# robertknight/ocrs

Measured on AMD Instinct MI355X. Metric: pages/sec end-to-end (1024x1024), higher is better.
Workload: dtype f32

## Files before the change

### include/ocrs_amd.h

```cpp
#ifndef OCRS_AMD_H
#define OCRS_AMD_H

#include <stddef.h>
#include <stdint.h>

#if defined(__GNUC__)
#define OCRS_API __attribute__((visibility("default")))
#else
#define OCRS_API
#endif

#ifdef __cplusplus
extern "C" {
#endif

typedef enum ocrs_status {
    OCRS_OK = 0,
    OCRS_ERR_INVALID_ARGUMENT = 1,
    OCRS_ERR_MODEL_NOT_LOADED = 2,
    OCRS_ERR_MODEL_DIMS = 3,
    OCRS_ERR_RUN_FAILED = 4,
    OCRS_ERR_WRONG_OUTPUT = 5,
    OCRS_ERR_IMAGE_SOURCE = 6,
    OCRS_ERR_DEVICE = 7,
// ... 258 lines not shown

typedef struct ocrs_speckle_params {
    float threshold;
    int32_t max_area;
    int32_t max_hole;
    int32_t keep_near;
    float paper;
    float ink_level;
} ocrs_speckle_params;
typedef struct ocrs_speckle_info {
    int32_t paper_bin;
    int32_t ink_bin;
    float paper_fill;
    float ink_fill;
    uint64_t ink;
    uint64_t counted;
    uint64_t specks;
    uint64_t kept;
    uint64_t speck_pixels;
    uint64_t kept_pixels;
    uint64_t holes;
    uint64_t hole_pixels;
} ocrs_speckle_info;
OCRS_API ocrs_status ocrs_speckle_params_default(ocrs_speckle_params* out);
OCRS_API ocrs_status ocrs_speckle_params_check(const ocrs_speckle_params* params);
OCRS_API ocrs_status ocrs_engine_despeckle_page(const ocrs_engine* e, const ocrs_page* page, const ocrs_speckle_params* params,
                                                ocrs_page** out_page, uint8_t** out_mask, ocrs_speckle_info* out_info);
OCRS_API ocrs_status ocrs_engine_despeckle_pages(const ocrs_engine* e, const ocrs_page* const* pages, size_t n,
                                                 const ocrs_speckle_params* params, ocrs_page** out_pages, uint8_t** out_masks,
                                                 ocrs_speckle_info* out_infos);

OCRS_API float ocrs_engine_detection_threshold(const ocrs_engine* e);

OCRS_API ocrs_status ocrs_engine_find_text_lines(const ocrs_engine* e, const ocrs_page* page, const float* word_rects,
                                        size_t n_words, float** line_rects, size_t** line_offsets,
                                        size_t* n_lines);

OCRS_API ocrs_status ocrs_engine_find_text_lines_batch(const ocrs_engine* e, size_t n_pages, const float* word_rects,
                                                       const size_t* word_offsets, float** line_rects,
                                                       size_t** line_offsets, size_t** page_line_offsets);

OCRS_API ocrs_status ocrs_engine_find_text_lines_indexed(const ocrs_engine* e, const ocrs_page* page, const float* word_rects,
                                                         size_t n_words, float** line_rects, size_t** line_offsets,
                                                         size_t* n_lines, size_t** word_index);
OCRS_API ocrs_status ocrs_engine_find_text_lines_batch_indexed(const ocrs_engine* e, size_t n_pages, const float* word_rects,
                                                               const size_t* word_offsets, float** line_rects,
                                                               size_t** line_offsets, size_t** page_line_offsets,
                                                               size_t** word_index);

typedef struct ocrs_text_char {
    uint32_t ch;
    int32_t top, left, bottom, right;
} ocrs_text_char;

OCRS_API ocrs_status ocrs_engine_recognize_text(const ocrs_engine* e, const ocrs_page* page, const float* line_rects,
                                       const size_t* line_offsets, size_t n_lines, ocrs_text_char** chars,
                                       size_t** char_offsets);
OCRS_API ocrs_status ocrs_engine_recognize_text_batch(const ocrs_engine* e, const ocrs_page* const* pages, size_t n_pages,
                                             const size_t* page_line_offsets, const float* line_rects,
                                             const size_t* line_offsets, size_t n_lines,
                                             ocrs_text_char** chars, size_t** char_offsets);

OCRS_API ocrs_status ocrs_engine_recognize_text_scored(const ocrs_engine* e, const ocrs_page* page, const float* line_rects,
                                                       const size_t* line_offsets, size_t n_lines, ocrs_text_char** chars,
                                                       size_t** char_offsets, float** char_logp, double** line_score);
OCRS_API ocrs_status ocrs_engine_recognize_text_batch_scored(const ocrs_engine* e, const ocrs_page* const* pages,
                                                             size_t n_pages, const size_t* page_line_offsets,
                                                             const float* line_rects, const size_t* line_offsets,
                                                             size_t n_lines, ocrs_text_char** chars, size_t** char_offsets,
                                                             float** char_logp, double** line_score);

OCRS_API ocrs_status ocrs_engine_recognize_tokens(const ocrs_engine* e, const ocrs_page* page, const float* line_rects,
                                         const size_t* line_offsets, size_t n_lines, uint32_t** labels,
                                         uint32_t** positions, size_t** token_offsets);

OCRS_API ocrs_status ocrs_engine_recognize_logits(const ocrs_engine* e, const ocrs_page* page, const float* line_rects,
                                         const size_t* line_offsets, size_t n_lines, float** logp, size_t** row_offsets,
                                         int* classes);

OCRS_API ocrs_status ocrs_engine_run_recognition_ops(const ocrs_engine* e, const int32_t* line_widths, size_t n_lines, int first_op,
                                                     int last_op, int gx_only, const float* input, size_t input_len, float** out,
                                                     size_t** out_offsets, int32_t** out_shapes);

OCRS_API ocrs_status ocrs_text_item_rotated_rect(const int32_t* rects_tlbr, size_t n_chars, float out6[6]);
OCRS_API ocrs_status ocrs_rotated_rect_corners(const float rect6[6], float out8[8]);

OCRS_API ocrs_status ocrs_engine_prepare_recognition_input(const ocrs_engine* e, const ocrs_page* page, const float* line,
                                                  size_t n_words, float** out, int* height, int* width);

OCRS_API ocrs_status ocrs_line_frame(const float* words, size_t n_words, int rec_height, double axis[2], double extents[4],
                                     uint32_t* resized_width, float coef[6], int32_t* ranges, int* empty);
OCRS_API ocrs_status ocrs_line_char_boxes(const float* words, size_t n_words, int rec_height, uint32_t ctc_input_len,
                                          const uint32_t* positions, size_t n_steps, int32_t* rects_tlbr, uint8_t* kept);
OCRS_API ocrs_status ocrs_engine_prepare_recognition_input_rectified(const ocrs_engine* e, const ocrs_page* page, const float* line,
                                                                     size_t n_words, float** out, int* height, int* width);
OCRS_API ocrs_status ocrs_engine_recognize_text_rectified(const ocrs_engine* e, const ocrs_page* page, const float* line_rects,
                                                          const size_t* line_offsets, size_t n_lines, ocrs_text_char** chars,
                                                          size_t** char_offsets, float** char_logp, double** line_score);
OCRS_API ocrs_status ocrs_engine_recognize_text_batch_rectified(const ocrs_engine* e, const ocrs_page* const* pages, size_t n_pages,
                                                                const size_t* page_line_offsets, const float* line_rects,
                                                                const size_t* line_offsets, size_t n_lines, ocrs_text_char** chars,
                                                                size_t** char_offsets, float** char_logp, double** line_score);
OCRS_API ocrs_status ocrs_engine_recognize_tokens_rectified(const ocrs_engine* e, const ocrs_page* page, const float* line_rects,
                                                            const size_t* line_offsets, size_t n_lines, uint32_t** labels,
                                                            uint32_t** positions, size_t** token_offsets);

OCRS_API ocrs_status ocrs_engine_rotate_page(const ocrs_engine* e, const ocrs_page* page, int quarter_turns, ocrs_page** out);
OCRS_API ocrs_status ocrs_engine_rotate_pages(const ocrs_engine* e, const ocrs_page* const* pages, size_t n, const int* quarter_turns,
                                              ocrs_page** out);
OCRS_API ocrs_status ocrs_unrotate_rects(float* rects6, size_t n, int page_h, int page_w, int k);
OCRS_API ocrs_status ocrs_unrotate_chars(ocrs_text_char* chars, size_t n, int page_h, int page_w, int k);
OCRS_API ocrs_status ocrs_unwarp_chars(ocrs_text_char* chars, size_t n, const float m[6]);
OCRS_API ocrs_status ocrs_unproject_chars(ocrs_text_char* chars, size_t n, const float m[8]);
OCRS_API ocrs_status ocrs_orientation_vote(const float* rects6, size_t n, double out[2]);
OCRS_API ocrs_status ocrs_engine_detect_orientation(const ocrs_engine* e, const ocrs_page* page, size_t max_lines, int* quarter_turns,
                                                    double vote[2], double score[4], uint32_t n_chars[4]);

OCRS_API ocrs_status ocrs_engine_get_text(const ocrs_engine* e, const ocrs_page* page, char** text);

OCRS_API ocrs_status ocrs_engine_prepare_input_jpeg(const ocrs_engine* e, const void* jpeg, size_t len, ocrs_page** out,
                                                    size_t* coef_bytes);
OCRS_API ocrs_status ocrs_jpeg_decode_rgb(int device, const void* jpeg, size_t len, uint8_t** rgb, int* height, int* width,
                                          size_t* coef_bytes);
OCRS_API ocrs_status ocrs_jpeg_info(const void* jpeg, size_t len, int* height, int* width, int* components, int* progressive,
                                    size_t* nonzero);
OCRS_API ocrs_status ocrs_jpeg_coefficients(const void* jpeg, size_t len, int32_t geom[28], uint16_t quant[256], int16_t** coef,
                                            size_t* n_blocks);

typedef struct ocrs_engine_group ocrs_engine_group;
typedef enum ocrs_gather_mode { OCRS_GATHER_AUTO = 0, OCRS_GATHER_HOST = 1, OCRS_GATHER_RCCL = 2 } ocrs_gather_mode;

typedef struct ocrs_group_params {
    const void* detection_model;
    size_t detection_model_len;
    const void* recognition_model;
    size_t recognition_model_len;
    const int* devices;
    size_t n_devices;
    int debug;
    ocrs_decode_method decode_method;
    uint32_t beam_width;
    const char* alphabet;
    const char* allowed_chars;
    ocrs_gather_mode gather;
    ocrs_numerics numerics;
    int coalesce, coalesce_pages, coalesce_window_us, layout_threads;
    int64_t rec_max_pixels;
    int min_block;
    int shared_block;
} ocrs_group_params;

OCRS_API ocrs_status ocrs_engine_group_new(const ocrs_group_params* params, ocrs_engine_group** out);
OCRS_API void ocrs_engine_group_free(ocrs_engine_group* g);
OCRS_API ocrs_status ocrs_engine_group_size(const ocrs_engine_group* g, size_t* n_members);
OCRS_API ocrs_status ocrs_engine_group_member(const ocrs_engine_group* g, size_t i, const ocrs_engine** engine, int* device);
OCRS_API ocrs_status ocrs_group_deal(size_t n_pages, size_t n_members, size_t min_block, size_t* member_of_page, size_t* pages_per_member);

OCRS_API ocrs_status ocrs_group_prepare_input_batch(const ocrs_engine_group* g, const void* const* pixels, size_t n,
                                                    ocrs_pixel_type type, ocrs_dim_order order, int height, int width,
                                                    int channels, ocrs_page** out);
OCRS_API ocrs_status ocrs_group_prepare_input_device_batch(const ocrs_engine_group* g, const void* const* d_pixels, size_t n,
                                                           ocrs_pixel_type type, ocrs_dim_order order, int height, int width,
                                                           int channels, ocrs_page** out);
OCRS_API ocrs_status ocrs_group_detect_words_batch(ocrs_engine_group* g, const ocrs_page* const* pages, size_t n_pages,
                                                   float** rects, size_t* offsets);
OCRS_API ocrs_status ocrs_group_detect_words_batch_scored(ocrs_engine_group* g, const ocrs_page* const* pages, size_t n_pages,
// ... 49 lines not shown
```

### ocrs_amd/__init__.py

```python
import ctypes as C
import math

import numpy as np

from . import _lib
from ._lib import OcrsError, check, lib

__all__ = ["OcrEngine", "OcrEngineParams", "ImageSource", "ImageSourceError", "DimOrder", "DecodeMethod", "Model",
           "OcrInput", "TextLine", "TextWord", "TextChar", "OcrsError", "DEFAULT_ALPHABET", "EngineGroup", "line_frame",
           "Orientation", "orientation_vote", "unrotate_rects", "unrotate_lines", "work_size", "rescale_rects", "normalize_params", "rules_params", "speckle_params"]

DEFAULT_ALPHABET = " 0123456789!\"#$%&'()*+,-./:;<=>?@[\\]^_`{|}~€ABCDEFGHIJKLMNOPQRSTUVWXYZabcdefghijklmnopqrstuvwxyz"


class DimOrder:
    Hwc = 0
    Chw = 1


class DecodeMethod:
    Greedy = ("greedy", 0)

    @staticmethod
    def BeamSearch(width):
# ... 1110 lines not shown
        chars = C.POINTER(_lib.TextCharC)()
        coffs = C.POINTER(C.c_size_t)()
        args = [self._h, pages, C.c_size_t(n), plo_a.ctypes.data_as(C.POINTER(C.c_size_t)),
                rects.ctypes.data_as(C.POINTER(C.c_float)), offs.ctypes.data_as(C.POINTER(C.c_size_t)),
                C.c_size_t(len(all_lines)), C.byref(chars), C.byref(coffs)]
        clp = lsc = None
        if scores:
            clp, lsc = C.POINTER(C.c_float)(), C.POINTER(C.c_double)()
        if rectify:
            check(lib().ocrs_engine_recognize_text_batch_rectified(*args, C.byref(clp) if scores else None,
                                                                   C.byref(lsc) if scores else None))
        elif scores:
            check(lib().ocrs_engine_recognize_text_batch_scored(*args, C.byref(clp), C.byref(lsc)))
        else:
            check(lib().ocrs_engine_recognize_text_batch(*args))
        result = []
        li = 0
        for lines in lines_per_page:
            page_out = []
            for _ in lines:
                page_out.append(_line_from_c(chars, coffs, clp, lsc, li))
                li += 1
            result.append(page_out)
        for p in (chars, coffs, clp, lsc):
            if p is not None:
                lib().ocrs_buffer_free(p)
        return result

    def recognize_tokens(self, inp, lines, rectify=False):
        rects, offs = _pack_lines(lines)
        lab = C.POINTER(C.c_uint32)()
        pos = C.POINTER(C.c_uint32)()
        toff = C.POINTER(C.c_size_t)()
        fn = lib().ocrs_engine_recognize_tokens_rectified if rectify else lib().ocrs_engine_recognize_tokens
        check(fn(self._h, inp._h, rects.ctypes.data_as(C.POINTER(C.c_float)),
                 offs.ctypes.data_as(C.POINTER(C.c_size_t)), C.c_size_t(len(lines)), C.byref(lab), C.byref(pos), C.byref(toff)))
        out = []
        for i in range(len(lines)):
            out.append([(int(lab[k]), int(pos[k])) for k in range(toff[i], toff[i + 1])])
        for p in (lab, pos, toff):
            lib().ocrs_buffer_free(p)
        return out

    def recognize_logits(self, inp, lines):
        rects, offs = _pack_lines(lines)
        lp = C.POINTER(C.c_float)()
        roff = C.POINTER(C.c_size_t)()
        ncls = C.c_int(0)
        check(lib().ocrs_engine_recognize_logits(self._h, inp._h, rects.ctypes.data_as(C.POINTER(C.c_float)),
                                                 offs.ctypes.data_as(C.POINTER(C.c_size_t)), C.c_size_t(len(lines)),
                                                 C.byref(lp), C.byref(roff), C.byref(ncls)))
        c = ncls.value
        out = []
        for i in range(len(lines)):
            a, b = roff[i], roff[i + 1]
            out.append(np.ctypeslib.as_array(lp, shape=(roff[len(lines)] * c,))[a * c:b * c].reshape(b - a, c).copy() if b > a
                       else np.zeros((0, c), np.float32))
        lib().ocrs_buffer_free(lp)
        lib().ocrs_buffer_free(roff)
        return out

    def run_recognition_ops(self, widths, first_op, last_op, inputs, gx_only=False):
        w = np.ascontiguousarray(widths, np.int32)
        flat = np.ascontiguousarray(np.concatenate([np.asarray(a, np.float32).ravel() for a in inputs]), np.float32)
        out = C.POINTER(C.c_float)()
        offs = C.POINTER(C.c_size_t)()
        shp = C.POINTER(C.c_int32)()
        check(lib().ocrs_engine_run_recognition_ops(self._h, w.ctypes.data_as(C.POINTER(C.c_int32)), C.c_size_t(len(w)),
                                                    int(first_op), int(last_op), int(bool(gx_only)),
                                                    flat.ctypes.data_as(C.POINTER(C.c_float)), C.c_size_t(flat.size),
                                                    C.byref(out), C.byref(offs), C.byref(shp)))
        n = len(w)
        res = []
        for i in range(n):
            a, b = offs[i], offs[i + 1]
            d = (shp[3 * i], shp[3 * i + 1], shp[3 * i + 2])
            v = np.ctypeslib.as_array(out, shape=(max(offs[n], 1),))[a:b].copy() if b > a else np.zeros(0, np.float32)
            res.append(v.reshape(d))
        lib().ocrs_buffer_free(out)
        lib().ocrs_buffer_free(offs)
        lib().ocrs_buffer_free(shp)
        return res

    def prepare_recognition_input(self, inp, line, rectify=False):
        a = _rects_to_array(line)
        out = C.POINTER(C.c_float)()
        h, w = C.c_int(0), C.c_int(0)
        fn = lib().ocrs_engine_prepare_recognition_input_rectified if rectify else lib().ocrs_engine_prepare_recognition_input
        check(fn(self._h, inp._h, a.ctypes.data_as(C.POINTER(C.c_float)), C.c_size_t(len(a)), C.byref(out), C.byref(h), C.byref(w)))
        img = np.ctypeslib.as_array(out, shape=(max(h.value * w.value, 1),))[: h.value * w.value].reshape(h.value, w.value).copy()
        lib().ocrs_buffer_free(out)
        return img

    def detection_threshold(self):
        return float(lib().ocrs_engine_detection_threshold(self._h))

    def get_text(self, inp, rectify=False, orientation=None, work_size=None, normalize=None, deskew=None, deskew_fill=0.5,
                 perspective=None, perspective_fill=0.5, rules=None, despeckle=None):
        if perspective is not None:
            inp = self.straighten(inp, None if isinstance(perspective, str) and perspective == "auto" else perspective, fill=perspective_fill)[0]
        if normalize is not None and normalize is not False:
            inp = self.normalize(inp, **({} if normalize is True else dict(normalize)))
        if despeckle is not None and despeckle is not False:
            inp = self.despeckle(inp, **({} if despeckle is True else dict(despeckle)))
        if orientation is not None:
            k = self.detect_orientation(inp).quarter_turns if orientation == "auto" else int(orientation)
            inp = self.rotate(inp, k)
        if deskew is not None:
            inp = self.deskew(inp, None if deskew == "auto" else float(deskew), fill=deskew_fill)[0]
        if rules is not None and rules is not False:
            inp = self.remove_rules(inp, **({} if rules is True else dict(rules)))
        if work_size is not None or rectify:
            lines = self.find_text_lines(inp, self.detect_words(inp, work_size=work_size))
            return "\n".join(str(t) for t in self.recognize_text(inp, lines, rectify=rectify) if t is not None)
        txt = C.c_char_p()
        check(lib().ocrs_engine_get_text(self._h, inp._h, C.byref(txt)))
        s = txt.value.decode("utf-8")
        lib().ocrs_buffer_free(txt)
        return s

    def enable_timing(self, level=1):
        check(lib().ocrs_engine_enable_timing(self._h, int(level)))

    def set_kernel_timing_classes(self, names=None):
        n = lib().ocrs_kernel_class_count()
        all_names = [lib().ocrs_kernel_class_name(i).decode() for i in range(n)]
        mask = 0xFFFFFFFF if names is None else sum(1 << all_names.index(x) for x in names)
        check(lib().ocrs_engine_set_kernel_timing_mask(self._h, C.c_uint32(mask)))

    def kernel_stats(self, reset=True):
        n = lib().ocrs_kernel_class_count()
        ms = (C.c_double * n)()
        cnt = (C.c_uint64 * n)()
        fl = (C.c_double * n)()
        by = (C.c_double * n)()
        mf = (C.c_double * n)()
        check(lib().ocrs_engine_kernel_mfma_flops(self._h, mf))
        check(lib().ocrs_engine_kernel_stats(self._h, ms, cnt, fl, by, 1 if reset else 0))
        return {lib().ocrs_kernel_class_name(i).decode(): dict(ms=ms[i], launches=int(cnt[i]), flops=fl[i], bytes=by[i],
                                                               mfma_flops=mf[i])
                for i in range(n)}

    def stage_times(self, reset=True):
        n = lib().ocrs_stage_count()
        ms = (C.c_double * n)()
        cnt = (C.c_uint64 * n)()
        check(lib().ocrs_engine_stage_times(self._h, ms, cnt, 1 if reset else 0))
        return {lib().ocrs_stage_name(i).decode(): (ms[i], int(cnt[i])) for i in range(n)}

    def __del__(self):
        try:
            if self._h and getattr(self, "_owned", True):
                lib().ocrs_engine_free(self._h)
            self._h = None
        except Exception:
            pass


def _line_from_c(chars, coffs, clp, lsc, li):
    a, b = coffs[li], coffs[li + 1]
    if b <= a:
        return None
    return TextLine([TextChar(chr(chars[k].ch), (chars[k].top, chars[k].left, chars[k].bottom, chars[k].right),
                              None if clp is None else np.float32(clp[k])) for k in range(a, b)],
                    None if lsc is None else float(lsc[li]))

# ... 158 lines not shown
```

### ocrs_amd/_lib.py

```python
import ctypes as C
import os

_HERE = os.path.dirname(os.path.abspath(__file__))
LIB_PATH = os.environ.get("OCRS_AMD_LIB") or os.path.join(_HERE, "libocrs_amd.so")

OCRS_OK = 0
STATUS_NAMES = {
    0: "OK", 1: "INVALID_ARGUMENT", 2: "MODEL_NOT_LOADED", 3: "MODEL_DIMS", 4: "RUN_FAILED", 5: "WRONG_OUTPUT",
    6: "IMAGE_SOURCE", 7: "DEVICE", 8: "IO", 9: "CAPACITY",
}

RUN_FN = C.CFUNCTYPE(C.c_int, C.c_void_p, C.POINTER(C.c_float), C.POINTER(C.c_int64), C.POINTER(C.POINTER(C.c_float)),
                     C.POINTER(C.c_int64), C.POINTER(C.c_int))


class EngineParams(C.Structure):
    _fields_ = [("detection_model", C.c_void_p), ("recognition_model", C.c_void_p), ("debug", C.c_int),
                ("decode_method", C.c_int), ("beam_width", C.c_uint32), ("alphabet", C.c_char_p),
                ("allowed_chars", C.c_char_p), ("numerics", C.c_int), ("coalesce", C.c_int), ("coalesce_pages", C.c_int),
                ("coalesce_window_us", C.c_int), ("layout_threads", C.c_int), ("rec_max_pixels", C.c_int64)]


class GroupParams(C.Structure):
    _fields_ = [("detection_model", C.c_void_p), ("detection_model_len", C.c_size_t), ("recognition_model", C.c_void_p),
                ("recognition_model_len", C.c_size_t), ("devices", C.POINTER(C.c_int)), ("n_devices", C.c_size_t),
                ("debug", C.c_int), ("decode_method", C.c_int), ("beam_width", C.c_uint32), ("alphabet", C.c_char_p),
                ("allowed_chars", C.c_char_p), ("gather", C.c_int), ("numerics", C.c_int), ("coalesce", C.c_int),
                ("coalesce_pages", C.c_int), ("coalesce_window_us", C.c_int), ("layout_threads", C.c_int), ("rec_max_pixels", C.c_int64),
                ("min_block", C.c_int), ("shared_block", C.c_int)]


class RunOptions(C.Structure):
    _fields_ = [("timing", C.c_int)]


class TextCharC(C.Structure):
    _fields_ = [("ch", C.c_uint32), ("top", C.c_int32), ("left", C.c_int32), ("bottom", C.c_int32),
                ("right", C.c_int32)]


class OcrsError(RuntimeError):
    def __init__(self, status, message):
        super().__init__(message)
        self.status = status
        self.status_name = STATUS_NAMES.get(status, str(status))


DECLARED_SYMBOLS = [
    "ocrs_last_error", "ocrs_buffer_free", "ocrs_device_count", "ocrs_set_device", "ocrs_set_option", "ocrs_ctc_beam_search", "ocrs_model_load_file",
    "ocrs_model_load_bytes", "ocrs_model_from_callback", "ocrs_model_input_shape", "ocrs_model_run",
    "ocrs_model_flops", "ocrs_model_free", "ocrs_engine_new", "ocrs_engine_free", "ocrs_image_source_check_bytes",
    "ocrs_engine_prepare_input", "ocrs_engine_prepare_input_device", "ocrs_page_free", "ocrs_page_dims",
    "ocrs_page_image", "ocrs_engine_detect_words", "ocrs_engine_detect_words_batch",
    "ocrs_engine_detect_text_pixels", "ocrs_engine_detection_threshold", "ocrs_engine_find_text_lines",
    "ocrs_engine_find_text_lines_batch",
    "ocrs_engine_recognize_text", "ocrs_engine_recognize_text_batch", "ocrs_engine_recognize_tokens",
    "ocrs_engine_prepare_recognition_input", "ocrs_text_item_rotated_rect", "ocrs_rotated_rect_corners", "ocrs_engine_get_text", "ocrs_device_malloc", "ocrs_device_free",
    "ocrs_device_upload", "ocrs_device_synchronize", "ocrs_device_measure_peaks", "ocrs_engine_enable_timing", "ocrs_stage_count",
    "ocrs_stage_name", "ocrs_engine_stage_times", "ocrs_kernel_class_count", "ocrs_kernel_class_name",
    "ocrs_engine_kernel_stats", "ocrs_engine_set_kernel_timing_mask", "ocrs_gru_tile_plan", "ocrs_host_malloc", "ocrs_host_free", "ocrs_engine_prepare_input_batch",
    "ocrs_get_device", "ocrs_model_load_file_on_device", "ocrs_model_load_bytes_on_device", "ocrs_model_device", "ocrs_engine_device",
    "ocrs_engine_group_new", "ocrs_engine_group_free", "ocrs_engine_group_size", "ocrs_engine_group_member", "ocrs_group_deal",
    "ocrs_group_prepare_input_batch", "ocrs_group_prepare_input_device_batch", "ocrs_group_detect_words_batch",
    "ocrs_group_recognize_text_batch", "ocrs_group_gather", "ocrs_group_final_gather", "ocrs_group_worker_threads", "ocrs_group_last_gather", "ocrs_device_malloc_on", "ocrs_engine_coalesce_stats", "ocrs_coalescer_selftest", "ocrs_stream_plan_selftest", "ocrs_conv_rows_selftest", "ocrs_engine_kernel_mfma_flops", "ocrs_engine_prepare_input_jpeg", "ocrs_jpeg_decode_rgb", "ocrs_jpeg_info", "ocrs_jpeg_coefficients",
    "ocrs_group_member_stats", "ocrs_numa_parse_cpulist", "ocrs_numa_bind_selftest", "ocrs_engine_recognize_logits", "ocrs_engine_set_option", "ocrs_engine_get_option", "ocrs_option_name", "ocrs_device_pool_stats", "ocrs_device_pool_configure", "ocrs_device_pool_trim",
    "ocrs_device_set_isolation", "ocrs_device_isolation", "ocrs_group_set_replay", "ocrs_abi_version",
    "ocrs_engine_recognize_text_scored", "ocrs_engine_recognize_text_batch_scored", "ocrs_ctc_beam_search_scored",
    "ocrs_engine_run_recognition_ops",
    "ocrs_engine_detect_words_scored", "ocrs_engine_detect_words_batch_scored", "ocrs_group_detect_words_batch_scored",
    "ocrs_engine_find_text_lines_indexed", "ocrs_engine_find_text_lines_batch_indexed",
    "ocrs_detection_tile_plan", "ocrs_engine_detect_words_tiled", "ocrs_engine_detect_words_batch_tiled",
    "ocrs_engine_detect_text_pixels_tiled", "ocrs_group_detect_words_batch_tiled",
    "ocrs_line_frame", "ocrs_line_char_boxes", "ocrs_engine_prepare_recognition_input_rectified",
    "ocrs_engine_recognize_text_rectified", "ocrs_engine_recognize_text_batch_rectified",
    "ocrs_group_recognize_text_batch_rectified", "ocrs_engine_recognize_tokens_rectified",
    "ocrs_engine_rotate_page", "ocrs_engine_rotate_pages", "ocrs_unrotate_rects", "ocrs_unrotate_chars",
    "ocrs_orientation_vote", "ocrs_engine_detect_orientation", "ocrs_engine_page_from_grey",
    "ocrs_engine_resize_page", "ocrs_engine_resize_pages", "ocrs_work_size", "ocrs_rescale_rects",
    "ocrs_engine_detect_words_at", "ocrs_engine_detect_words_batch_at",
    "ocrs_normalize_params_default", "ocrs_normalize_params_check", "ocrs_engine_normalize_page", "ocrs_engine_normalize_pages",
    "ocrs_skew_params_default", "ocrs_skew_params_check", "ocrs_skew_table", "ocrs_engine_skew_scores", "ocrs_engine_estimate_skew",
    "ocrs_engine_warp_page", "ocrs_engine_warp_pages", "ocrs_deskew_map", "ocrs_unwarp_rects", "ocrs_unwarp_chars",
    "ocrs_outline_params_default", "ocrs_outline_params_check", "ocrs_engine_edge_peaks", "ocrs_outline_choose", "ocrs_engine_find_outline",
    "ocrs_quad_map", "ocrs_engine_project_page", "ocrs_engine_project_pages", "ocrs_unproject_rects", "ocrs_unproject_chars",
    "ocrs_rules_params_default", "ocrs_rules_params_check", "ocrs_engine_remove_rules_page", "ocrs_engine_remove_rules_pages",
    "ocrs_speckle_params_default", "ocrs_speckle_params_check", "ocrs_engine_despeckle_page", "ocrs_engine_despeckle_pages",
]

ABI_VERSION = 6
TILE_OVERLAP_DEFAULT = 100
RESAMPLE_FILTERS = {"auto": 0, "bilinear": 1, "area": 2}
POLARITIES = {"auto": 0, "keep": 1, "invert": 2}


class NormalizeParams(C.Structure):
    _fields_ = [("tile", C.c_int32), ("polarity", C.c_int32), ("flatten", C.c_int32), ("levels", C.c_int32)]


class NormalizeInfo(C.Structure):
    _fields_ = [("dark", C.c_int32), ("white", C.c_int32), ("lo", C.c_int32), ("hi", C.c_int32), ("vote", C.c_int64),
                ("counted", C.c_uint64)]

    def as_dict(self):
        return {"dark": int(self.dark), "vote": int(self.vote), "white": int(self.white), "lo": int(self.lo), "hi": int(self.hi),
                "counted": int(self.counted)}


class RulesParams(C.Structure):
    _fields_ = [("threshold", C.c_float), ("min_length", C.c_int32), ("max_thickness", C.c_int32), ("margin", C.c_int32), ("paper", C.c_float)]


class RulesInfo(C.Structure):
    _fields_ = [("paper_bin", C.c_int32), ("fill", C.c_float), ("ink", C.c_uint64), ("counted", C.c_uint64), ("h_removed", C.c_uint64),
                ("v_removed", C.c_uint64), ("overwritten", C.c_uint64), ("kept", C.c_uint64)]

    def as_dict(self):
        return {"paper_bin": int(self.paper_bin), "fill": float(self.fill), "ink": int(self.ink), "counted": int(self.counted),
                "h_removed": int(self.h_removed), "v_removed": int(self.v_removed), "overwritten": int(self.overwritten),
                "kept": int(self.kept)}


class SpeckleParams(C.Structure):
    _fields_ = [("threshold", C.c_float), ("max_area", C.c_int32), ("max_hole", C.c_int32), ("keep_near", C.c_int32), ("paper", C.c_float),
                ("ink_level", C.c_float)]


class SpeckleInfo(C.Structure):
    _fields_ = [("paper_bin", C.c_int32), ("ink_bin", C.c_int32), ("paper_fill", C.c_float), ("ink_fill", C.c_float), ("ink", C.c_uint64),
                ("counted", C.c_uint64), ("specks", C.c_uint64), ("kept", C.c_uint64), ("speck_pixels", C.c_uint64),
                ("kept_pixels", C.c_uint64), ("holes", C.c_uint64), ("hole_pixels", C.c_uint64)]

    def as_dict(self):
        return {name: (float if name.endswith("_fill") else int)(getattr(self, name)) for name, _ in self._fields_}


class SkewParams(C.Structure):
    _fields_ = [("max_deg", C.c_double), ("coarse_step_deg", C.c_double), ("fine_step_deg", C.c_double), ("work_max_side", C.c_int32),
                ("reserved", C.c_int32)]


class SkewInfo(C.Structure):
    _fields_ = [("angle_deg", C.c_double), ("best_score", C.c_uint64), ("second_score", C.c_uint64), ("fine_score", C.c_uint64),
                ("work_h", C.c_int32), ("work_w", C.c_int32), ("coarse_index", C.c_int32), ("fine_index", C.c_int32)]


class OutlineParams(C.Structure):
    _fields_ = [("max_deg", C.c_double), ("step_deg", C.c_double), ("min_cover", C.c_double), ("min_span", C.c_double), ("min_area", C.c_double),
                ("work_max_side", C.c_int32), ("min_step", C.c_int32)]


class OutlineInfo(C.Structure):
# ... 160 lines not shown
```

### ocrs_amd/csrc/abi.cpp

```cpp
#include <cstdio>
#include <fstream>
#include <thread>

#include <atomic>
#include "abi_util.hpp"
#include "coalesce_selftest.hpp"
#include "conv_rows.hpp"
#include "engine.hpp"
#include "host_pool.hpp"
#include "jpeg.hpp"
#include "kernels.hpp"
#include "page_ops.hpp"

using namespace ocrs;
using namespace ocrs::geom;

using namespace ocrs::abi;

extern "C" {

const char* ocrs_last_error(void) { return last_error().c_str(); }

void ocrs_buffer_free(void* p) { free(p); }

// ... 849 lines not shown
        const LineFrame f = line_frame(words, n_words, rec_height);
        for (size_t i = 0; i < n_steps; i++) {
            kept[i] = 0;
            for (int q = 0; q < 4; q++) rects_tlbr[4 * i + q] = 0;
        }
        for (const auto& kv : rectified_char_boxes(f, (f.rw + 49) / 50 * 50, ctc_input_len, positions, n_steps)) {
            kept[kv.first] = 1;
            const int32_t r[4] = {kv.second.top, kv.second.left, kv.second.bottom, kv.second.right};
            std::copy(r, r + 4, rects_tlbr + 4 * kv.first);
        }
    });
}

static ocrs_status recognize_tokens(const ocrs_engine* e, const ocrs_page* page, const float* line_rects,
                                    const size_t* line_offsets, size_t n_lines, uint32_t** labels,
                                    uint32_t** positions, size_t** token_offsets, bool rectify) {
    return guarded_engine(e, [&] {
        if (!e || !page || !line_offsets || !labels || !positions || !token_offsets)
            fail(OCRS_ERR_INVALID_ARGUMENT, "null argument");
        check_pages_on(e, &page, 1);
        std::vector<std::vector<std::vector<RotatedRect>>> lpp(1);
        lpp[0] = unpack_lines(line_rects, line_offsets, 0, n_lines);
        std::vector<RecResult> res;
        e->recognize(&page, 1, lpp, &res, false, rectify);
        std::vector<uint32_t> fl, fp;
        std::vector<size_t> offs{0};
        for (const RecResult& r : res) {
            for (const CtcStep& c : r.steps) { fl.push_back(c.label); fp.push_back(c.pos); }
            offs.push_back(fl.size());
        }
        *labels = dup_buffer(fl);
        *positions = dup_buffer(fp);
        *token_offsets = dup_buffer(offs);
    });
}

ocrs_status ocrs_engine_recognize_tokens(const ocrs_engine* e, const ocrs_page* page, const float* line_rects,
                                         const size_t* line_offsets, size_t n_lines, uint32_t** labels,
                                         uint32_t** positions, size_t** token_offsets) {
    return recognize_tokens(e, page, line_rects, line_offsets, n_lines, labels, positions, token_offsets, false);
}

ocrs_status ocrs_engine_recognize_tokens_rectified(const ocrs_engine* e, const ocrs_page* page, const float* line_rects,
                                                   const size_t* line_offsets, size_t n_lines, uint32_t** labels,
                                                   uint32_t** positions, size_t** token_offsets) {
    return recognize_tokens(e, page, line_rects, line_offsets, n_lines, labels, positions, token_offsets, true);
}

ocrs_status ocrs_engine_recognize_logits(const ocrs_engine* e, const ocrs_page* page, const float* line_rects,
                                         const size_t* line_offsets, size_t n_lines, float** logp, size_t** row_offsets, int* classes) {
    return guarded_engine(e, [&] {
        if (!e || !page || !line_offsets || !logp || !row_offsets || !classes) fail(OCRS_ERR_INVALID_ARGUMENT, "null argument");
        check_pages_on(e, &page, 1);
        std::vector<std::vector<float>> per_line;
        e->recognize_logits(page, unpack_lines(line_rects, line_offsets, 0, n_lines), &per_line, classes);
        std::vector<float> flat;
        std::vector<size_t> offs{0};
        for (const auto& l : per_line) {
            flat.insert(flat.end(), l.begin(), l.end());
            offs.push_back(flat.size() / (size_t)*classes);
        }
        *logp = dup_buffer(flat);
        *row_offsets = dup_buffer(offs);
    });
}

ocrs_status ocrs_engine_run_recognition_ops(const ocrs_engine* e, const int32_t* line_widths, size_t n_lines, int first_op,
                                            int last_op, int gx_only, const float* input, size_t input_len, float** out,
                                            size_t** out_offsets, int32_t** out_shapes) {
    return guarded_engine(e, [&] {
        if (!e || !line_widths || !input || !out || !out_offsets || !out_shapes) fail(OCRS_ERR_INVALID_ARGUMENT, "null argument");
        std::vector<float> flat;
        std::vector<int32_t> shapes;
        e->run_recognition_ops(line_widths, n_lines, first_op, last_op, gx_only != 0, input, input_len, &flat, &shapes);
        std::vector<size_t> offs{0};
        for (size_t i = 0; i < n_lines; i++)
            offs.push_back(offs.back() + (size_t)shapes[3 * i] * shapes[3 * i + 1] * shapes[3 * i + 2]);
        *out = dup_buffer(flat);
        *out_offsets = dup_buffer(offs);
        *out_shapes = dup_buffer(shapes);
    });
}

ocrs_status ocrs_text_item_rotated_rect(const int32_t* rects_tlbr, size_t n_chars, float out6[6]) {
    return guarded([&] {
        if (!rects_tlbr || !out6 || n_chars == 0) fail(OCRS_ERR_INVALID_ARGUMENT, "expected valid rect");
        RotatedRect rr;
        if (!text_item_rotated_rect(rects_tlbr, n_chars, &rr)) fail(OCRS_ERR_INVALID_ARGUMENT, "expected valid rect");
        rr.to_array(out6);
    });
}

ocrs_status ocrs_rotated_rect_corners(const float rect6[6], float out8[8]) {
    return guarded([&] {
        if (!rect6 || !out8) fail(OCRS_ERR_INVALID_ARGUMENT, "null argument");
        auto c = RotatedRect::from_array(rect6).corners();
        for (int i = 0; i < 4; i++) { out8[2 * i] = c[i].x; out8[2 * i + 1] = c[i].y; }
    });
}

static ocrs_status prepare_recognition_input(const ocrs_engine* e, const ocrs_page* page, const float* line, size_t n_words, float** out,
                                             int* height, int* width, bool rectify) {
    return guarded_engine(e, [&] {
        if (!e || !page || !line || !out || !height || !width) fail(OCRS_ERR_INVALID_ARGUMENT, "null argument");
        check_pages_on(e, &page, 1);
        if (!e->recognition) fail(OCRS_ERR_MODEL_NOT_LOADED, "Recognition model not loaded");
        const RecLine ln = e->make_rec_line(unpack_words(line, n_words), 0, 0, rectify);
        const int rec_h = (int)e->rec_input_height();
        const int rw = (int)ln.resized_width, cw = rectify ? (int)ln.group_width : rw;
        std::vector<float> host((size_t)rec_h * rw);
        if (rw > 0) {
            Workspace ws;
            const float* d_out = stage_line_crops(ws, nullptr, &page, 1, {CropLine{&ln, (uint32_t)cw, 0}}, rec_h, (int64_t)rec_h * cw);
            if (cw == rw) {
                ws.download(host.data(), d_out, host.size() * 4);
                ws.sync();
            } else {
                std::vector<float> full((size_t)rec_h * cw);
                ws.download(full.data(), d_out, full.size() * 4);
                ws.sync();
                for (int y = 0; y < rec_h; y++) std::copy_n(&full[(size_t)y * cw], rw, &host[(size_t)y * rw]);
            }
        }
        *out = dup_buffer(host);
        *height = rec_h;
        *width = rw;
    });
}

ocrs_status ocrs_engine_prepare_recognition_input(const ocrs_engine* e, const ocrs_page* page, const float* line,
                                                  size_t n_words, float** out, int* height, int* width) {
    return prepare_recognition_input(e, page, line, n_words, out, height, width, false);
}

ocrs_status ocrs_engine_prepare_recognition_input_rectified(const ocrs_engine* e, const ocrs_page* page, const float* line,
                                                            size_t n_words, float** out, int* height, int* width) {
    return prepare_recognition_input(e, page, line, n_words, out, height, width, true);
}

ocrs_status ocrs_engine_get_text(const ocrs_engine* e, const ocrs_page* page, char** text) {
    return guarded_engine(e, [&] {
        if (!e || !page || !text) fail(OCRS_ERR_INVALID_ARGUMENT, "null argument");
        check_pages_on(e, &page, 1);
        std::vector<std::vector<RotatedRect>> rr;
        e->detect(&page, 1, &rr, nullptr);
        std::vector<std::vector<std::vector<RotatedRect>>> lpp(1);
        lpp[0] = find_text_lines(rr[0]);
        std::vector<RecResult> res;
        e->recognize(&page, 1, lpp, &res);
        std::string out;
        bool first = true;
        for (const RecResult& r : res) {
            auto chars = e->text_line_from_result(r);
            if (chars.empty()) continue;
            if (!first) out.push_back('\n');
            first = false;
            for (const TextChar& c : chars) append_utf8(out, c.ch);
        }
        char* p = static_cast<char*>(malloc(out.size() + 1));
        if (!p) throw std::bad_alloc();
        memcpy(p, out.c_str(), out.size() + 1);
        *text = p;
    });
}

ocrs_status ocrs_device_malloc(size_t bytes, void** d_ptr) {
// ... 91 lines not shown
```

### ocrs_amd/csrc/common.cpp

```cpp
#include "common.hpp"

#include <chrono>
#include <climits>
#include <cstdint>
#include <cstdlib>
#include <cstring>

#include <algorithm>
#include <atomic>
#include <condition_variable>
#include <deque>
#include <system_error>

namespace ocrs {

static thread_local std::string g_last_error;

void set_last_error(const std::string& msg) { g_last_error = msg; }
const std::string& last_error() { return g_last_error; }

namespace {
std::atomic<int> g_default_device{0};
thread_local DeviceContext* t_ctx = nullptr;
constexpr int kMaxDevices = 64;
// ... 394 lines not shown
    return relaxed_;
}

int DeviceContext::cu_count() {
    std::lock_guard<std::mutex> g(lazy_mu_);
    if (!cus_) {
        hipDeviceProp_t prop;
        OCRS_HIP(hipGetDeviceProperties(&prop, device));
        cus_ = prop.multiProcessorCount;
    }
    return cus_;
}

namespace {
struct OptDef { const char* name; const char* env; long def; };
const OptDef kOptDefs[OPT_COUNT] = {
    {"gru_mode", "OCRS_GRU_MODE", GRU_PERSISTENT},
    {"gru_gates", "OCRS_GRU_GATES", 1},
    {"gru_local", "OCRS_GRU_LOCAL", 1},
    {"det_fuse", "OCRS_DET_FUSE", 1},
    {"det_stream", "OCRS_DET_STREAM", 1},
    {"det_rows", "OCRS_DET_ROWS", 1},
    {"ccl_quad", "OCRS_CCL_QUAD", 1},
    {"conv12_fuse", "OCRS_CONV12_FUSE", 1},
    {"conv_flat", "OCRS_CONV_FLAT", 1},
    {"beam_gpu", "OCRS_BEAM_GPU", 1},
    {"det_tile_batch", "OCRS_DET_TILE_BATCH", 16},
    {"stream_budget", "OCRS_STREAM_BUDGET", LanePlan::kDefaultBudget},
    {"numerics", nullptr, 0},
    {"coalesce", nullptr, 2},
    {"coalesce_pages", nullptr, 16},
    {"coalesce_window_us", nullptr, 300},
    {"layout_threads", nullptr, 0},
    {"rec_max_pixels", nullptr, 0},
};
struct OptRange { long lo, hi; long also[4]; };
const OptRange kOptRanges[OPT_COUNT] = {
    {0, 1, {}}, {0, 1, {}}, {0, 1, {}}, {0, 2, {}}, {0, 1, {8, 14, 32}}, {0, 1, {8, 14, 20, 32}}, {0, 1, {}}, {0, 1, {}}, {0, 1, {}}, {0, 1, {}},
    {1, 1024, {}}, {LanePlan::kMinBudget, LanePlan::kMaxBudget, {}},
    {0, 2, {}}, {0, 64, {}}, {1, 4096, {}}, {0, 10000000, {}}, {0, 4096, {}}, {0, INT64_MAX, {}},
};
bool in_range(int i, long v) {
    const OptRange& r = kOptRanges[i];
    if (i == OPT_STREAM_BUDGET) return LanePlan::valid_budget(v);
    if (v >= r.lo && v <= r.hi) return true;
    for (long a : r.also) if (a && v == a) return true;
    return false;
}
const char* const kRetired[] = {"det_heavy", "det_tail", "gru_waves", "gru_background", "gru_scatter", "gru_gates_pack", "conv_occupancy",
                                "gx_heavy", "gemm_nfast", "conv_a_lds", "gru_heavy", "heavy_priority", "det_mfma"};
std::atomic<long> g_opts[OPT_COUNT];
std::once_flag g_opts_once;
void init_options() {
    for (int i = 0; i < OPT_COUNT; i++) {
        const char* e = kOptDefs[i].env ? getenv(kOptDefs[i].env) : nullptr;
        const long v = e && *e ? strtol(e, nullptr, 10) : kOptDefs[i].def;
        g_opts[i].store(in_range(i, v) ? v : kOptDefs[i].def);
    }
}
int find_option(const char* name, int count = OPT_PUBLIC_COUNT) {
    for (int i = 0; i < count; i++)
        if (name && i != OPT_NUMERICS && strcmp(name, kOptDefs[i].name) == 0) return i;
    return -1;
}
thread_local const Tuning* t_tuning = nullptr;
}

TuningScope::TuningScope(const Tuning* t) : prev_(t_tuning) { t_tuning = t; }
TuningScope::~TuningScope() { t_tuning = prev_; }
const Tuning* current_tuning() { return t_tuning; }

long process_option(Option o) {
    std::call_once(g_opts_once, init_options);
    return g_opts[o].load(std::memory_order_relaxed);
}

long option_long(Option o) {
    if (t_tuning) return __atomic_load_n(&t_tuning->v[o], __ATOMIC_RELAXED);
    std::call_once(g_opts_once, init_options);
    return g_opts[o].load(std::memory_order_relaxed);
}
int option(Option o) { return (int)option_long(o); }
int conv_rows_setting() { return t_tuning ? (int)__atomic_load_n(&t_tuning->conv_rows, __ATOMIC_RELAXED) : (int)kConvRowsDefault; }

Tuning default_tuning() {
    std::call_once(g_opts_once, init_options);
    Tuning t;
    for (int i = 0; i < OPT_COUNT; i++) t.v[i] = g_opts[i].load(std::memory_order_relaxed);
    t.conv_rows = kConvRowsDefault;
    return t;
}

const char* option_name(int i) { return i >= 0 && i < OPT_PUBLIC_COUNT ? kOptDefs[i].name : nullptr; }

int set_option(const char* name, long value) {
    std::call_once(g_opts_once, init_options);
    const int i = find_option(name);
    if (i < 0) {
        for (const char* r : kRetired) if (name && strcmp(name, r) == 0) return 0;
        return 1;
    }
    if (!in_range(i, value)) return 2;
    if (i == OPT_STREAM_BUDGET && value != g_opts[i].load() && any_device_has_calls_in_flight()) return 3;
    g_opts[i].store(value);
    return 0;
}

int set_option(Tuning& t, const char* name, long value) {
    if (name && strcmp(name, "conv_rows") == 0) {
        if (value < 0 || value > 2) return 2;
        __atomic_store_n(&t.conv_rows, value, __ATOMIC_RELAXED);
        return 0;
    }
    const int i = find_option(name, OPT_COUNT);
    if (i < 0) return 1;
    if (i == OPT_STREAM_BUDGET) return 4;
    if (!in_range(i, value)) return 2;
    __atomic_store_n(&t.v[i], value, __ATOMIC_RELAXED);
    return 0;
}

bool get_option(const Tuning& t, const char* name, long* value) {
    if (name && strcmp(name, "conv_rows") == 0) {
        *value = __atomic_load_n(&t.conv_rows, __ATOMIC_RELAXED);
        return true;
    }
    const int i = name && strcmp(name, "numerics") == 0 ? (int)OPT_NUMERICS : find_option(name, OPT_COUNT);
    if (i < 0) return false;
    *value = __atomic_load_n(&t.v[i], __ATOMIC_RELAXED);
    return true;
}

static hipEvent_t take_lease_event(DeviceContext* c) {
    {
        std::lock_guard<std::mutex> g(c->stream_mu);
        if (!c->lease_events.empty()) {
            hipEvent_t e = c->lease_events.back();
            c->lease_events.pop_back();
            return e;
        }
    }
    hipEvent_t e = nullptr;
    OCRS_HIP(hipEventCreateWithFlags(&e, hipEventBlockingSync | hipEventDisableTiming));
    return e;
}

StreamLease::StreamLease(bool high_priority, int avoid_lane) : ctx_(&ctx()), high_(high_priority) {
    high_ = true;
    mode_ = ctx_->lease_begin();
    try {
        done_ = take_lease_event(ctx_);
        if (mode_ == DeviceContext::MODE_SERIAL) {
            s_ = ctx_->heavy_stream();
            shared_ = true;
            return;
        }
        (void)ctx_->planned_light_lanes();
        lane_ = ctx_->plan.acquire(avoid_lane);
        counted_ = true;
        if (lane_ >= 0) {
            s_ = ctx_->light_lane(lane_);
            return;
        }
        {
            std::lock_guard<std::mutex> g(ctx_->stream_mu);
            auto& v = ctx_->streams;
            if (!v.empty()) {
                s_ = v.back();
                v.pop_back();
                return;
            }
        }
        int least = 0, greatest = 0;
        OCRS_HIP(hipDeviceGetStreamPriorityRange(&least, &greatest));
        OCRS_HIP(hipStreamCreateWithPriority(&s_, hipStreamNonBlocking, greatest));
    } catch (...) {
        if (counted_) ctx_->plan.release(lane_);
        if (done_) {
            std::lock_guard<std::mutex> g(ctx_->stream_mu);
            ctx_->lease_events.push_back(done_);
        }
        ctx_->lease_end();
        throw;
    }
}

StreamLease::~StreamLease() {
    {
        std::lock_guard<std::mutex> g(ctx_->stream_mu);
        ctx_->lease_events.push_back(done_);
        if (!shared_ && lane_ < 0) ctx_->streams.push_back(s_);
    }
    if (counted_) ctx_->plan.release(lane_);
    ctx_->lease_end();
}

std::vector<StageTimers::Pending>& StageTimers::pending() {
    static thread_local std::vector<Pending> p;
    return p;
}
std::map<int, std::vector<hipEvent_t>>& StageTimers::thread_events() {
    static thread_local std::map<int, std::vector<hipEvent_t>> f;
    return f;
}
std::vector<hipEvent_t>& StageTimers::free_events() { return thread_events()[ctx().device]; }

hipEvent_t StageTimers::get_event() {
// ... 71 lines not shown
```

### ocrs_amd/csrc/common.hpp

```cpp
#pragma once
#include <atomic>
#include <hip/hip_runtime.h>

#include <cstdarg>
#include <cstdint>
#include <cstdio>
#include <cstdlib>
#include <chrono>
#include <condition_variable>
#include <cstring>
#include <map>
#include <mutex>
#include <stdexcept>
#include <string>
#include <thread>
#include <vector>

#include "../../include/ocrs_amd.h"
#include "stream_plan.hpp"

namespace ocrs {

struct Error : std::runtime_error {
    ocrs_status status;
// ... 48 lines not shown
    void release(void* p);
    void set_cap(uint64_t bytes);
    PoolStats stats();

  private:
    std::mutex mu_;
    std::multimap<size_t, void*> free_;
    std::map<void*, size_t> live_;
    uint64_t cached_ = 0, live_bytes_ = 0, peak_live_ = 0, cap_ = uint64_t(1) << 30, allocs_ = 0;
    std::atomic<uint64_t> frees_{0};
};

struct DeviceContext {
    const int device;
    DevicePool pool;
    HostPool host_pool;
    std::mutex heavy_phase, rec_phase;
    hipStream_t heavy_stream();
    hipStream_t recurrent_stream(int mode = 0);
    enum Isolation { ISO_AUTO = 0, ISO_NONE = 1 };
    enum Mode { MODE_FREE = 0, MODE_SERIAL = 1 };
    Mode lease_begin();
    void lease_end();
    void add_relaxed_engine(int delta);
    void set_isolation(Isolation policy);
    Mode current_mode();
    int relaxed_engine_count();
    int cu_count();
    std::vector<struct DevBuf> heavy_arena;
    std::mutex stream_mu;
    LanePlan plan;
    std::vector<hipStream_t> streams;
    std::vector<hipEvent_t> lease_events;
    hipStream_t light_lane(int lane);
    int planned_light_lanes();
    bool calls_in_flight();

    explicit DeviceContext(int d) : device(d), pool(d) {}

  private:
    Mode mode_locked() const { return policy_ == ISO_NONE || relaxed_ <= 0 ? MODE_FREE : MODE_SERIAL; }
    template <class F> void switch_isolation(F&& change);
    std::mutex lazy_mu_;
    hipStream_t heavy_ = nullptr, recurrent_ = nullptr;
    std::vector<hipStream_t> light_;
    void create_lanes_locked(int n_light);
    int cus_ = 0;
    std::mutex iso_mu_;
    std::condition_variable iso_cv_;
    int leases_ = 0, relaxed_ = 0;
    bool switching_ = false;
    Isolation policy_ = ISO_AUTO;
    friend class StreamLease;
};

DeviceContext& device_context(int device);
int default_device();
void select_device(int device);
DeviceContext& ctx();

class DeviceScope {
  public:
    explicit DeviceScope(int device);
    ~DeviceScope();
    DeviceScope(const DeviceScope&) = delete;
    DeviceScope& operator=(const DeviceScope&) = delete;

  private:
    DeviceContext* prev_;
    int restore_ = -1;
};

inline DevicePool& pool() { return ctx().pool; }
inline HostPool& host_pool() { return ctx().host_pool; }
inline hipStream_t heavy_stream() { return ctx().heavy_stream(); }

enum Option { OPT_GRU_MODE = 0, OPT_GRU_GATES, OPT_GRU_LOCAL, OPT_DET_FUSE, OPT_DET_STREAM, OPT_DET_ROWS, OPT_CCL_QUAD,
              OPT_CONV12_FUSE, OPT_CONV_FLAT, OPT_BEAM_GPU, OPT_DET_TILE_BATCH, OPT_STREAM_BUDGET, OPT_PUBLIC_COUNT,
              OPT_NUMERICS = OPT_PUBLIC_COUNT,
              OPT_COALESCE, OPT_COALESCE_PAGES, OPT_COALESCE_WINDOW_US,
              OPT_LAYOUT_THREADS, OPT_REC_MAX_PIXELS,
              OPT_COUNT };
constexpr long kConvRowsDefault = 2;
struct Tuning { long v[OPT_COUNT]; long conv_rows; };
int conv_rows_setting();
Tuning default_tuning();
int set_option(const char* name, long value);
int set_option(Tuning& t, const char* name, long value);
bool get_option(const Tuning& t, const char* name, long* value);
const char* option_name(int i);
class TuningScope {
  public:
    explicit TuningScope(const Tuning* t);
    ~TuningScope();
    TuningScope(const TuningScope&) = delete;
    TuningScope& operator=(const TuningScope&) = delete;
  private:
    const Tuning* prev_;
};
const Tuning* current_tuning();
enum { GRU_PERSISTENT = 0, GRU_STEP = 1 };
int option(Option o);
long process_option(Option o);

inline void allow_dynamic_lds(const void* kernel, std::atomic<uint64_t>& done) {
    int dev = 0;
    (void)hipGetDevice(&dev);
    const uint64_t bit = 1ull << (dev & 63);
    if (done.load(std::memory_order_relaxed) & bit) return;
    (void)hipFuncSetAttribute(kernel, hipFuncAttributeMaxDynamicSharedMemorySize, 160 * 1024);
    done.fetch_or(bit, std::memory_order_relaxed);
}
long option_long(Option o);
inline int gru_mode() { return option(OPT_GRU_MODE); }

struct DevBuf {
    void* p = nullptr;
    size_t bytes = 0;
    DevicePool* owner = nullptr;
    DevBuf() = default;
    explicit DevBuf(size_t n) : bytes(n), owner(n ? &pool() : nullptr) { p = n ? owner->alloc(n) : nullptr; }
    DevBuf(const DevBuf&) = delete;
    DevBuf& operator=(const DevBuf&) = delete;
    DevBuf(DevBuf&& o) noexcept : p(o.p), bytes(o.bytes), owner(o.owner) { o.p = nullptr; o.bytes = 0; o.owner = nullptr; }
    DevBuf& operator=(DevBuf&& o) noexcept {
        if (this != &o) { reset(); p = o.p; bytes = o.bytes; owner = o.owner; o.p = nullptr; o.bytes = 0; o.owner = nullptr; }
        return *this;
    }
    ~DevBuf() { reset(); }
    void reset() { if (p && owner) owner->release(p); p = nullptr; bytes = 0; owner = nullptr; }
    int device() const { return owner ? owner->device() : -1; }
    template <class T> T* as() const { return static_cast<T*>(p); }
};

struct PinnedBuf {
    void* p = nullptr;
    size_t bytes = 0;
    PinnedBuf() = default;
    explicit PinnedBuf(size_t n) : bytes(n) { if (n) OCRS_HIP(hipHostMalloc(&p, n, hipHostMallocPortable)); }
    PinnedBuf(const PinnedBuf&) = delete;
    PinnedBuf& operator=(const PinnedBuf&) = delete;
    ~PinnedBuf() { if (p) (void)hipHostFree(p); }
    template <class T> T* as() const { return static_cast<T*>(p); }
};

inline hipError_t wait_event(hipEvent_t ev) noexcept {
    for (int i = 0;; i++) {
        const hipError_t e = hipEventQuery(ev);
        if (e != hipErrorNotReady) return e;
        if (i < 64) std::this_thread::yield();
        else std::this_thread::sleep_for(std::chrono::microseconds(i < 256 ? 20 : 100));
    }
}

class StreamLease {
  public:
    explicit StreamLease(bool high_priority = false, int avoid_lane = LanePlan::kPrivate);
    ~StreamLease();
    hipStream_t get() const { return s_; }
    int lane() const { return lane_; }
    bool may_park_waits() const { return lane_ < 0 || ctx_->plan.outstanding() <= 1; }
    hipError_t wait_done() const noexcept {
        const hipError_t e = hipEventRecord(done_, s_);
        return e != hipSuccess ? e : wait_event(done_);
    }
    void sync() const { OCRS_HIP(wait_done()); }
    hipError_t sync_noexcept() const noexcept { return wait_done(); }
    DeviceContext::Mode mode() const { return mode_; }
// ... 136 lines not shown
```

### ocrs_amd/csrc/engine.cpp

```cpp
#include "engine.hpp"

#include <algorithm>
#include <exception>
#include <limits>
#include <map>
#include <thread>

#include "kernels.hpp"

using namespace ocrs;
using namespace ocrs::geom;

TileAxisPlan ocrs::tile_axis_plan(int L, int M, int v) {
    if (L <= 0 || M <= 0 || v < 0 || v > M / 2) fail(OCRS_ERR_INVALID_ARGUMENT, "tile plan: length %d, model length %d, overlap %d", L, M, v);
    TileAxisPlan p;
    if (L <= M) {
        p.origin = {0};
        p.bound = {0, L};
        return p;
    }
    const int n = (L - v + (M - v) - 1) / (M - v);
    p.origin.resize(n);
    p.bound.resize(n + 1);
    for (int i = 0; i < n; i++) p.origin[i] = (int32_t)(((int64_t)i * (L - M)) / (n - 1));
// ... 827 lines not shown
    const std::vector<int32_t>& hoff = plan.h_off;

    const bool seq_in = first_op > ts;
    const int in_c = shp[0][in_slot].c;
    std::vector<float> packed;
    std::vector<size_t> line_at(n);
    {
        size_t acc = 0;
        for (size_t i = 0; i < n; i++) {
            if (shp[i][in_slot].c != in_c) fail(OCRS_ERR_INVALID_ARGUMENT, "op %d: input channels differ between lines", first_op);
            line_at[i] = acc;
            acc += (size_t)shp[i][in_slot].count();
        }
        if (acc != in_len) fail(OCRS_ERR_INVALID_ARGUMENT, "input has %zu floats, op %d of these lines reads %zu", in_len, first_op, acc);
    }
    if (seq_in) {
        packed.resize((size_t)plan.R * in_c);
        for (size_t i = 0; i < n; i++)
            for (int t = 0; t < T[i]; t++)
                std::copy_n(in + line_at[i] + (size_t)t * in_c, in_c, &packed[((size_t)hoff[t] + slot_of[i]) * in_c]);
    } else {
        for (size_t i : order) packed.insert(packed.end(), in + line_at[i], in + line_at[i] + shp[i][in_slot].count());
    }

    float* d_in = ws.alloc_n<float>(std::max<size_t>(packed.size(), 1));
    ws.upload(d_in, packed.data(), packed.size() * sizeof(float));
    std::vector<HipModel::PackedGroup> pg;
    {
        size_t at = 0, pos = 0;
        for (auto& kv : by_w) {
            const size_t ng = kv.second.size();
            pg.push_back(HipModel::PackedGroup{d_in + (seq_in ? 0 : at), (int)ng, (int)kv.first, d_pos + pos});
            for (size_t i : kv.second) at += (size_t)shp[i][in_slot].count();
            pos += ng;
        }
    }
    int32_t* d_labels = ws.alloc_n<int32_t>((size_t)plan.R);
    HipModel::OpRange r;
    r.first = first_op;
    r.last = last_op;
    r.gx_only = gx_only;
    r.seq_in = seq_in ? d_in : nullptr;
    r.in_c = in_c;
    hm->run_recognition_packed(ws, pg, plan, h, nullptr, nullptr, d_labels, nullptr, nullptr, &r);

    const bool seq_out = last_op >= ts;
    const int oc = r.out_c;
    std::vector<float> host;
    if (seq_out) {
        host.resize((size_t)(gx_only ? 2 : 1) * plan.R * oc);
    } else {
        size_t total = 0;
        for (size_t i = 0; i < n; i++) total += (size_t)shp[i][out_slot].count();
        host.resize(total);
    }
    ws.download(host.data(), r.out, host.size() * sizeof(float));
    ws.sync();
    for (uint32_t st8 : status)
        if (st8) fail(OCRS_ERR_DEVICE, "GRU recurrence kernel timed out waiting for a peer workgroup (status 0x%x)", st8);
    out->clear();
    shapes->clear();
    if (seq_out) {
        for (size_t i = 0; i < n; i++) {
            for (int d = 0; d < (gx_only ? 2 : 1); d++)
                for (int t = 0; t < T[i]; t++) {
                    const float* row = &host[((size_t)d * plan.R + hoff[t] + slot_of[i]) * oc];
                    out->insert(out->end(), row, row + oc);
                }
            shapes->insert(shapes->end(), gx_only ? std::initializer_list<int32_t>{2, T[i], oc} : std::initializer_list<int32_t>{T[i], 1, oc});
        }
    } else {
        std::vector<size_t> at(n);
        size_t acc = 0;
        for (size_t i : order) { at[i] = acc; acc += (size_t)shp[i][out_slot].count(); }
        for (size_t i = 0; i < n; i++) {
            const TensorShape& s = shp[i][out_slot];
            if (s.c != oc) fail(OCRS_ERR_RUN_FAILED, "op %d: %d output channels, the model says %d", last_op, oc, s.c);
            out->insert(out->end(), host.begin() + at[i], host.begin() + at[i] + s.count());
            shapes->insert(shapes->end(), {s.h, s.w, s.c});
        }
    }
}

namespace {

struct Chunk { uint32_t gw; std::vector<size_t> members; int64_t off; float* ptr = nullptr; };

void check_rec_output(int ndim, int64_t batch, size_t lines, int classes, size_t alphabet_len) {
    if (ndim != 3)
        fail(OCRS_ERR_WRONG_OUTPUT,
             "model output had unexpected type or shape: expected recognition output to have 3 dims but it has %d", ndim);
    if ((size_t)batch != lines)
        fail(OCRS_ERR_WRONG_OUTPUT, "model output had unexpected type or shape: batch size %lld != %zu", (long long)batch, lines);
    if (alphabet_len + 1 != (size_t)classes)
        fail(OCRS_ERR_WRONG_OUTPUT,
             "model output had unexpected type or shape: output column count (%d) does not match alphabet size (%zu)",
             classes, alphabet_len + 1);
}

struct DecodedSteps {
    int stride = 0;
    std::vector<uint32_t> hl, hp;
    std::vector<int32_t> hc;
    std::vector<float> hlp;
    std::vector<double> hscore;
};

void download_steps(Workspace& w, hipStream_t st, size_t M, int stride, const uint32_t* d_ol, const uint32_t* d_op, const int32_t* d_cnt,
                    const float* d_slp, const double* d_score, DecodedSteps* d) {
    d->stride = stride;
    d->hl.resize(M * stride);
    d->hp.resize(M * stride);
    d->hc.resize(M);
    w.download(d->hl.data(), d_ol, d->hl.size() * 4, st);
    w.download(d->hp.data(), d_op, d->hp.size() * 4, st);
    w.download(d->hc.data(), d_cnt, M * 4, st);
    if (d_slp) {
        d->hlp.resize(M * stride);
        d->hscore.resize(M);
        w.download(d->hlp.data(), d_slp, d->hlp.size() * sizeof(float), st);
        w.download(d->hscore.data(), d_score, M * sizeof(double), st);
    }
}

void take_steps(const DecodedSteps& d, size_t m, uint32_t ctc_len, RecResult* r) {
    const size_t at = m * d.stride;
    r->steps.resize(d.hc[m]);
    for (int q = 0; q < d.hc[m]; q++) r->steps[q] = CtcStep{d.hl[at + q], d.hp[at + q]};
    r->ctc_len = ctc_len;
    if (!d.hscore.empty()) {
        r->step_logp.assign(d.hlp.data() + at, d.hlp.data() + at + d.hc[m]);
        r->line_score = d.hscore[m];
    }
}

template <class Row>
void beam_decode_line(const ocrs_engine& e, int T, int C, Row row, std::vector<float>& seq, bool scored, RecResult* r) {
    seq.resize((size_t)T * C);
    for (int t = 0; t < T; t++) {
        const float* src = row(t);
        for (int c = 0; c < C; c++)
            seq[(size_t)t * C + c] = (e.has_excluded && e.excluded[c]) ? -std::numeric_limits<float>::infinity() : src[c];
    }
    double bs = 0.0;
    r->steps = ctc_beam_search(seq.data(), T, C, C, e.beam_width, scored ? &bs : nullptr);
    r->ctc_len = (uint32_t)T;
    if (scored) score_line(seq.data(), T, C, C, nullptr, r->steps, &bs, &r->step_logp, &r->line_score);
}

void recognize_callback(const ocrs_engine& e, Workspace& ws, const std::vector<Chunk>& chunks, RecResult* res, bool scored) {
    const auto* cb = static_cast<const CallbackModel*>(e.recognition);
    const bool beam = e.decode_method == OCRS_DECODE_BEAM_SEARCH;
    const uint32_t rec_h = e.rec_input_height();
    const uint8_t* d_excl = e.has_excluded ? e.d_excluded.as<uint8_t>() : nullptr;
    hipStream_t st = ws.s();
    std::vector<float> seq;
    for (const Chunk& ch : chunks) {
        const size_t nb = ch.members.size();
        const uint32_t gw = ch.gw;
        std::vector<float> hin(nb * rec_h * gw), hout;
        ws.download(hin.data(), ch.ptr, hin.size() * sizeof(float));
        ws.sync();
        const int64_t ishape[4] = {(int64_t)nb, 1, rec_h, gw};
        int64_t oshape[4] = {0, 0, 0, 0};
        int ond = 0;
        cb->run(hin.data(), ishape, hout, oshape, &ond);
// ... 288 lines not shown
```

### ocrs_amd/csrc/engine.hpp

```cpp
#pragma once
#include <string>
#include <vector>

#include <memory>

#include "coalesce.hpp"
#include "common.hpp"
#include "geometry.hpp"
#include "model.hpp"

struct ocrs_page {
    ocrs::DevBuf grey;
    int h = 0, w = 0;
    const void* source = nullptr;
    int device() const { return grey.device(); }
};

namespace ocrs {

struct CtcStep { uint32_t label, pos; };

std::vector<CtcStep> ctc_beam_search(const float* logp, int T, int C, int row_stride, uint32_t width, double* score = nullptr);
std::vector<CtcStep> ctc_beam_search_reference(const float* logp, int T, int C, int row_stride, uint32_t width,
                                               double* score = nullptr);
// ... 41 lines not shown
struct CropLine {
    const RecLine* line;
    uint32_t out_w;
    int64_t out_off;
};
float* stage_line_crops(Workspace& ws, StageTimers* timers, const ocrs_page* const* pages, size_t n_pages,
                        const std::vector<CropLine>& crops, int rec_h, int64_t total);

struct DetScores {
    std::vector<std::vector<float>> score;
    std::vector<std::vector<uint32_t>> pixels;
};

struct TileAxisPlan {
    std::vector<int32_t> origin;
    std::vector<int32_t> bound;
};
TileAxisPlan tile_axis_plan(int L, int M, int v);

struct DetRequest : CoalescedBase {
    const ocrs_page* const* pages = nullptr;
    size_t n = 0;
    std::vector<std::vector<geom::RotatedRect>>* rects = nullptr;
    DetScores* scores = nullptr;
};
struct RecRequest : CoalescedBase {
    const ocrs_page* const* pages = nullptr;
    size_t n_pages = 0;
    const std::vector<std::vector<std::vector<geom::RotatedRect>>>* lines_per_page = nullptr;
    std::vector<RecResult>* results = nullptr;
    bool scored = false;
    bool rectify = false;
};

}

struct ocrs_engine {
    int device = 0;
    const ocrs::ModelBase* detection = nullptr;
    const ocrs::ModelBase* recognition = nullptr;
    bool debug = false;
    ocrs_decode_method decode_method = OCRS_DECODE_GREEDY;
    uint32_t beam_width = 100;
    std::u32string alphabet;
    bool has_excluded = false;
    std::vector<uint8_t> excluded;
    ocrs::DevBuf d_excluded;
    float min_area = 100.0f;
    float text_threshold = 0.2f;
    mutable ocrs::StageTimers timers;
    ocrs::Tuning tuning{};
    ocrs::DeviceContext* counted_relaxed = nullptr;
    void count_relaxed(ocrs::DeviceContext& c) { uncount_relaxed(); c.add_relaxed_engine(+1); counted_relaxed = &c; }
    void uncount_relaxed() noexcept {
        if (!counted_relaxed) return;
        try { counted_relaxed->add_relaxed_engine(-1); } catch (...) {}
        counted_relaxed = nullptr;
    }
    ~ocrs_engine() { uncount_relaxed(); }

    ocrs::StageTimers* tm() const { return timers.enabled ? &timers : nullptr; }

    void detect(const ocrs_page* const* pages, size_t n, std::vector<std::vector<ocrs::geom::RotatedRect>>* rects,
                float* host_map , ocrs::DetScores* scores = nullptr, int tile_overlap = -1) const;
    void detect_now(const ocrs_page* const* pages, size_t n, std::vector<std::vector<ocrs::geom::RotatedRect>>* rects,
                    float* host_map, ocrs::DetScores* scores = nullptr, int tile_overlap = -1) const;

    void recognize(const ocrs_page* const* pages, size_t n_pages,
                   const std::vector<std::vector<std::vector<ocrs::geom::RotatedRect>>>& lines_per_page,
                   std::vector<ocrs::RecResult>* results, bool scored = false, bool rectify = false) const;
    void recognize_now(const ocrs_page* const* pages, size_t n_pages,
                       const std::vector<std::vector<std::vector<ocrs::geom::RotatedRect>>>& lines_per_page,
                       std::vector<ocrs::RecResult>* results, bool scored = false, bool want_logp = false,
                       const std::vector<char>* rectify_pages = nullptr) const;
    void init_coalescers();
    mutable std::unique_ptr<ocrs::Coalescer<ocrs::DetRequest>> det_queue;
    mutable std::unique_ptr<ocrs::Coalescer<ocrs::RecRequest>> rec_queue;
    void recognize_lines(const ocrs_page* const* pages, size_t n_pages, ocrs::RecResult* res, size_t n, bool scored,
                         bool want_logp) const;
    void recognize_logits(const ocrs_page* page, const std::vector<std::vector<ocrs::geom::RotatedRect>>& lines,
                          std::vector<std::vector<float>>* logp, int* classes) const;
    void run_recognition_ops(const int32_t* widths, size_t n, int first_op, int last_op, bool gx_only, const float* in,
                             size_t in_len, std::vector<float>* out, std::vector<int32_t>* shapes) const;

    std::vector<ocrs::TextChar> text_line_from_result(const ocrs::RecResult& res, std::vector<float>* char_logp = nullptr) const;

    uint32_t rec_input_height() const;
    ocrs::RecLine make_rec_line(const std::vector<ocrs::geom::RotatedRect>& words, size_t page, size_t index,
                                bool rectify = false) const;
};
```

### ocrs_amd/csrc/kernels.hpp

```cpp
#pragma once
#include <vector>
#include <hip/hip_runtime.h>

#include <cstdint>

namespace ocrs {
namespace jpeg { struct Coefficients; }
namespace k {

void prepare_image(const void* d_pixels, bool is_u8, bool chans_last, int h, int w, int chans, float* d_out,
                   hipStream_t s);
struct PrepareTable {
    enum { kPages = 32 };
    const void* src[kPages];
    float* dst[kPages];
};
void prepare_image_batch(const void* const* d_pixels, float* const* d_out, int n, bool is_u8, bool chans_last, int h, int w,
                         int chans, hipStream_t s);
void resize_pages_to_model(const float* const* d_src_ptrs, int n, int sh, int sw, int vh, int vw, float* d_dst,
                           int dh, int dw, hipStream_t s);
bool resize_threshold(const float* d_prob, int n, int mh, int mw, int sh, int sw, float thr, uint8_t* d_mask,
                      float* d_map, int h, int w, hipStream_t s, int32_t* d_labels = nullptr, int32_t* d_zero_a = nullptr,
                      int32_t* d_zero_b = nullptr);
void threshold_only(const float* d_prob, float thr, uint8_t* d_mask, int64_t count, hipStream_t s);

struct CclBuffers {
    int32_t* labels;
    int32_t* row_counts;
    int32_t* row_offsets;
    int32_t* n_roots;
    int32_t* roots;
    int32_t* lengths;
    int32_t* offsets;
    int32_t* overflow;
    uint32_t* pts;
    uint32_t* tmp;
    uint8_t* keep;
    float* rects;
    uint8_t* valid;
    uint32_t* score_pixels;
    unsigned long long* score_sums;
};
void ccl_label(const uint8_t* d_mask, int n, int h, int w, const CclBuffers& b, int max_comp, hipStream_t s, bool prepared = false);
void contour_rects(const uint8_t* d_mask, int n, int h, int w, const CclBuffers& b, int max_comp, int64_t arena,
                   float expand, float min_area, float eps, hipStream_t s, bool prepared = false);

void component_scores(const uint8_t* d_mask, const float* d_map, int n, int h, int w, const CclBuffers& b, int max_comp,
                      hipStream_t s);

struct TileDesc {
    const float* page;
    uint8_t* mask;
    float* map;
    int32_t h, w;
    int32_t oy, ox;
    int32_t y0, y1, x0, x1;
};
void gather_tiles(const TileDesc* d_tiles, int n_tiles, float* d_dst, int mh, int mw, hipStream_t s);
void stitch_threshold(const TileDesc* d_tiles, int n_tiles, const float* d_prob, int mh, int mw, float thr, hipStream_t s);

struct GemmDesc {
    const float* A; int lda;
    const float* B; int ldb;
    const float* bias;
    float* C; int ldc;
    int M, N, K;
    int relu;
    int im2col; int H, W, Cin;
    int convt; int Cout;
    int batch; int64_t strideA, strideB, strideBias, strideC;
    int nfast = 0, nx = 0, ny = 0;
    const uint16_t* Bsplit = nullptr; int64_t strideBsplit = 0;
};
void gemm(const GemmDesc& d, hipStream_t s);
void conv_direct(const float* x, int n, int h, int w, int cin, const float* wt, const float* bias, int kh, int kw,
                 int cout, int relu, float* y, hipStream_t s);
void dwconv3x3(const float* x, int n, int h, int w, int c, const float* wt, const float* bias, int relu, float* y,
               hipStream_t s);
bool dwpw_fused_supported(int cin, int cout);
void dwpw_fused(const float* x, int n, int h, int w, int cin, const float* wdw, const float* bdw, int relu_dw, int cout,
                const float* wpw, const float* bpw, int relu_pw, float* y, hipStream_t s);
bool dwconv3x3_cat(const float* skip, int n, int h, int w, int cs, const float* up, int uh, int uw, int cu, const float* wt,
                   const float* bias, int relu, float* y, hipStream_t s);
struct DoubleConvArgs {
    const float* skip;
    const float* x1;
    const float *wt, *bt;
    const float *wd1, *bd1;
    const float *wp1, *bp1;
    const float *wd2, *bd2;
    const float *wp2, *bp2;
    const float *wf, *bf;
    float* y;
    float* ypool;
    int n, h, w, h1, w1;
    int relu_d1, relu_p1, relu_d2, relu_p2, sigmoid;
    int tiles_x, tiles_y;
    const float* tape = nullptr;
    int tape_len = 0;
    const float* rtape = nullptr;
    int rtape_len = 0;
};
struct StreamWeights {
    const float *wt, *bt, *wd1, *bd1, *wp1, *bp1, *wd2, *bd2, *wp2, *bp2, *wf, *bf;
};
bool double_conv_fused(const DoubleConvArgs& a, int cs, int cx, int cmid, int cout, bool pool, bool final_conv,
                       bool launch, hipStream_t s, bool* on_mfma = nullptr, int* path = nullptr);
bool double_conv_stream(const DoubleConvArgs& a, int cs, int cx, int cmid, int cout, bool pool, bool final_conv, bool launch, hipStream_t s,
                        const StreamWeights* hw = nullptr, std::vector<float>* tape_out = nullptr, int* tape_len = nullptr);
bool double_conv_rows(const DoubleConvArgs& a, int cs, int cx, int cmid, int cout, bool pool, bool final_conv, bool launch, hipStream_t s,
                      const StreamWeights* hw = nullptr, std::vector<float>* tape_out = nullptr, int* tape_len = nullptr);
bool double_conv_rows_takes(const DoubleConvArgs& a, int cx);
void maxpool(const float* x, int n, int h, int w, int c, int kh, int kw, float* y, hipStream_t s);
void avgpool(const float* x, int n, int h, int w, int c, int kh, int kw, float* y, hipStream_t s);
void padcat(const float* skip, int n, int sh, int sw, int cs, const float* x, int h, int w, int cx, float* y,
            hipStream_t s);
void sigmoid(const float* x, float* y, int64_t count, hipStream_t s);
void conv1x1_cout1(const float* x, int64_t pixels, int cin, const float* wt, const float* bias, int relu, int do_sigmoid,
                   float* y, hipStream_t s);
void to_seq(const float* x, int n, int w, int c, float* y, hipStream_t s);
void gru_gates(const float* gx, const float* gh, float* h, float* y, int T, int N, int H, int step, hipStream_t s);
bool log_softmax_argmax(const float* logits, int64_t rows, int c, const uint8_t* d_excluded ,
                        float* logp, int32_t* labels, hipStream_t s, float* maxlp = nullptr);
void to_seq_packed(const float* x, int n, int T, int c, const int32_t* d_pos, const int32_t* d_off, float* y,
                   hipStream_t s);
void gru_gates_packed(const float* gx, const float* gh, float* h, float* y, const int32_t* d_Tm, const int32_t* d_off,
                      int64_t R, int Mcap, int active, int H, int step, hipStream_t s);
bool gru_step_fused(const float* gx, const float* wh, const float* bh, const float* hT_in, float* hT_out, float* y,
                    const int32_t* d_Tm, const int32_t* d_off, int64_t R, int Mcap, int active, int H, int step,
                    hipStream_t s);
size_t gru_persistent_sync_words(int M);
size_t gru_persistent_exchange_bytes(const int32_t* h_Tm, int M, int H);
bool gru_persistent_supported(const int32_t* h_Tm, int M, int Tmax, int64_t R, int H);
bool gru_tile_plan(const int32_t* h_Tm, int M, int H, int* ncl, int* waves, int16_t* tiles );
hipError_t gru_persistent_prepare(float* hx, const int32_t* h_Tm, int M, int H, hipStream_t s);
bool gru_persistent(const float* gx, const float* wh, const float* bh, float* y, float* hx, const int32_t* d_Tm, const int32_t* d_off,
                    const int32_t* h_Tm, int64_t R, int M, int Tmax, int H, uint32_t* d_sync, hipStream_t s);
bool gru_general_tile_plan(const int32_t* h_Tm, int M, int Tmax, int H, int cap, int* ncl, int16_t* tiles , int kernel );
size_t gru_split_exchange_bytes(const int32_t* h_Tm, int M, int H, int np);
bool gru_split_supported(const int32_t* h_Tm, int M, int Tmax, int64_t R, int H, int np);
hipError_t gru_split_prepare(uint16_t* hx, const int32_t* h_Tm, int M, int H, int np, hipStream_t s);
bool gru_persistent_split(const float* gx, const float* wh, const float* bh, float* y, uint16_t* hx, const int32_t* d_Tm, const int32_t* d_off,
                          const int32_t* h_Tm, int64_t R, int M, int Tmax, int H, int np, uint32_t* d_sync, hipStream_t s);
void ctc_collapse_packed(const int32_t* labels, const int32_t* d_Tm, const int32_t* d_off, int M, int Tmax,
                         uint32_t* out_labels, uint32_t* out_pos, int32_t* out_count, hipStream_t s);
void ctc_collapse_scored_packed(const int32_t* labels, const float* maxlp, const int32_t* d_Tm, const int32_t* d_off, int M,
                                int Tmax, uint32_t* out_labels, uint32_t* out_pos, float* out_logp, int32_t* out_count,
                                double* out_score, hipStream_t s);
void argmax_rows(const float* x, int64_t rows, int c, const uint8_t* d_excluded, int32_t* labels, hipStream_t s);
bool ctc_beam_supported(int C, int width);
size_t ctc_beam_arena_entries(int Tmax, int width);
bool ctc_beam_packed(const float* logp, const int32_t* d_Tm, const int32_t* d_off, int M, int Tmax, int C, int width,
                     const uint8_t* d_excluded, int2* d_nodes, int2* d_posn, uint32_t* out_labels, uint32_t* out_pos,
                     int32_t* out_count, hipStream_t s, double* out_score = nullptr, float* out_logp = nullptr);
void ctc_collapse(const int32_t* labels, int T, int N, uint32_t* out_labels, uint32_t* out_pos, int32_t* out_count,
                  hipStream_t s);

// ... 248 lines not shown
```

### ocrs_amd/csrc/kernels_nn.hip

```cpp
#include "common.hpp"
#include "kernels.hpp"
#include "split_mfma.hpp"
#include "spec_math.hpp"

namespace ocrs {
namespace k {

typedef float f32x16 __attribute__((ext_vector_type(16)));

constexpr int GEMM_BK = 32;

template <int NT, bool IM2COL, bool CONVT>
__global__ void __launch_bounds__(256) gemm_mfma_kernel(GemmDesc d) {
    extern __shared__ __attribute__((aligned(16))) float lds_b[];
    constexpr int BN = 32 * NT;
    const int tid = threadIdx.x;
    const int lane = tid & 63;
    const int wave = tid >> 6;
    const int half = lane >> 5;
    const int l31 = lane & 31;
    const int z = blockIdx.z;
    const float* __restrict__ A = d.A + (int64_t)z * d.strideA;
    const float* __restrict__ B = d.B + (int64_t)z * d.strideB;
    const float* __restrict__ bias = d.bias ? d.bias + (int64_t)z * d.strideBias : nullptr;
// ... 61 lines not shown

        for (int kk = 0; kk < kc; kk += 4) {
            float4 av = make_float4(0.f, 0.f, 0.f, 0.f);
            if (a_ok) {
                if (kk + 4 <= kc) {
                    av = *reinterpret_cast<const float4*>(arow + kk);
                } else {
                    av.x = arow[kk];
                    if (kk + 1 < kc) av.y = arow[kk + 1];
                    if (kk + 2 < kc) av.z = arow[kk + 2];
                }
            }
            const float a0 = half ? av.y : av.x;
            const float a1 = half ? av.w : av.z;
            const float* b0p = &lds_b[(kk + half) * BN + l31];
            const float* b1p = &lds_b[(kk + 2 + half) * BN + l31];
#pragma unroll
            for (int t = 0; t < NT; t++)
                acc[t] = __builtin_amdgcn_mfma_f32_32x32x2f32(a0, b0p[t * 32], acc[t], 0, 0, 0);
#pragma unroll
            for (int t = 0; t < NT; t++)
                acc[t] = __builtin_amdgcn_mfma_f32_32x32x2f32(a1, b1p[t * 32], acc[t], 0, 0, 0);
        }
    }

    const int64_t row_base = (int64_t)blockIdx.x * 128 + wave * 32;
#pragma unroll
    for (int t = 0; t < NT; t++) {
        const int col = n0 + t * 32 + l31;
        if (col >= d.N) continue;
#pragma unroll
        for (int r = 0; r < 16; r++) {
            const int64_t rr = row_base + (r & 3) + 8 * (r >> 2) + 4 * half;
            if (rr >= d.M) continue;
            float v = acc[t][r];
            if (d.relu) v = v > 0.0f ? v : 0.0f;
            if (CONVT) {
                int64_t hw = (int64_t)d.H * d.W;
                int64_t img = rr / hw;
                int rem = (int)(rr - img * hw);
                int y = rem / d.W, x = rem - y * d.W;
                int q = col / d.Cout, co = col - q * d.Cout;
                int dy = q >> 1, dx = q & 1;
                C[((img * 2 * d.H + 2 * y + dy) * (2 * (int64_t)d.W) + 2 * x + dx) * d.Cout + co] = v;
            } else {
                C[rr * d.ldc + col] = v;
            }
        }
    }
}

constexpr int TG_BM = 128, TG_BK = 16, TG_LDA = TG_BM + 1;

typedef float f32x4v __attribute__((ext_vector_type(4)));

template <int NTW, class Acc>
__device__ __forceinline__ void store_tile_rows(const Acc (&acc)[2][NTW], float* stage, int lane, bool relu, float* __restrict__ C,
                                                int64_t row0, int64_t M, int ldc) {
    constexpr int WN = 32 * NTW, LPR = WN / 4, RPI = 64 / LPR;
    const int half = lane >> 5, l31 = lane & 31;
    const int srow = lane / LPR, sc4 = (lane % LPR) * 4;
#pragma unroll
    for (int i = 0; i < 2; i++) {
#pragma unroll
        for (int t = 0; t < NTW; t++)
#pragma unroll
            for (int r = 0; r < 16; r++) {
                float v = acc[i][t][r];
                if (relu) v = v > 0.0f ? v : 0.0f;
                stage[((r & 3) + 8 * (r >> 2) + 4 * half) * WN + t * 32 + l31] = v;
            }
        asm volatile("s_waitcnt lgkmcnt(0)" ::: "memory");
#pragma unroll
        for (int it = 0; it < 32 / RPI; it++) {
            const int row = it * RPI + srow;
            const f32x4v v = *reinterpret_cast<const f32x4v*>(&stage[row * WN + sc4]);
            const int64_t rr = row0 + i * 32 + row;
            if (rr < M) *reinterpret_cast<f32x4v*>(&C[rr * ldc + sc4]) = v;
        }
        asm volatile("s_waitcnt lgkmcnt(0)" ::: "memory");
    }
}

template <int BN, bool IM2COL, bool PAIR>
__global__ void __launch_bounds__(256, 4) gemm_tiled_kernel(GemmDesc d) {
    extern __shared__ __attribute__((aligned(16))) float lds[];
    constexpr int NTW = BN / 64;
    float* As = lds;
    float* Bs = lds + 2 * TG_BK * TG_LDA;
    const int tid = threadIdx.x, lane = tid & 63, wave = tid >> 6;
    const int half = lane >> 5, l31 = lane & 31;
    const int wm = wave >> 1, wn = wave & 1;
    const int z = blockIdx.z;
    const float* __restrict__ A = d.A + (int64_t)z * d.strideA;
    const float* __restrict__ B = d.B + (int64_t)z * d.strideB;
    const float* __restrict__ bias = d.bias ? d.bias + (int64_t)z * d.strideBias : nullptr;
    float* __restrict__ C = d.C + (int64_t)z * d.strideC;
    int mblk, nblk;
    if (d.nfast) {
        const int xcd = blockIdx.x & 7, q = blockIdx.x >> 3;
        nblk = q % d.ny;
        mblk = (q / d.ny) * 8 + xcd;
        if (mblk >= d.nx) return;
    } else {
        const int nwg = gridDim.x, xcd = blockIdx.x & 7, xq = nwg >> 3, xr = nwg & 7;
        mblk = (xcd < xr ? xcd * (xq + 1) : xr * (xq + 1) + (xcd - xr) * xq) + (blockIdx.x >> 3);
        nblk = blockIdx.y;
    }
    const int64_t m0 = (int64_t)mblk * TG_BM;
    const int n0 = nblk * BN;

    constexpr int AQ = TG_BK / 4, AROWS = 256 / AQ, AV = TG_BM / AROWS;
    const int ar = tid / AQ, akq = tid % AQ;
    const float* arow_ptr[AV];
    int apy[AV], apx[AV];
#pragma unroll
    for (int j = 0; j < AV; j++) {
        int64_t row = m0 + ar + AROWS * j;
        if (row >= d.M) row = d.M - 1;
        if (IM2COL) {
            const int64_t hw = (int64_t)d.H * d.W;
            const int64_t img = row / hw;
            const int rem = (int)(row - img * hw);
            apy[j] = rem / d.W;
            apx[j] = rem - apy[j] * d.W;
            arow_ptr[j] = A + img * hw * d.Cin;
        } else {
            apy[j] = apx[j] = 0;
            arow_ptr[j] = A + row * d.lda;
        }
    }
    constexpr int BV = TG_BK * BN / 4 / 256;
    const bool b_vec = ((d.ldb & 3) == 0) && (((uintptr_t)B & 15) == 0);

    int boff[BV];
#pragma unroll
    for (int j = 0; j < BV; j++) {
        const int idx = tid + 256 * j;
        const int kk = idx / (BN / 4), nn = (idx % (BN / 4)) * 4;
        boff[j] = kk * d.ldb + min(n0 + nn, d.N - 4);
    }
    f32x4v pa[AV], pa2[AV], pb[BV];
    auto prefetch_b_fast = [&](int k0) {
        const float* __restrict__ bk = B + (int64_t)k0 * d.ldb;
#pragma unroll
        for (int j = 0; j < BV; j++) pb[j] = *reinterpret_cast<const f32x4v*>(bk + boff[j]);
    };
    auto prefetch_a_pair = [&](int k0) {
#pragma unroll
        for (int j = 0; j < AV; j++) {
            const float* src = arow_ptr[j] + k0 + akq * 4;
            pa[j] = *reinterpret_cast<const f32x4v*>(src);
            pa2[j] = *reinterpret_cast<const f32x4v*>(src + TG_BK);
        }
    };
    auto prefetch = [&](int k0) {
        if (IM2COL) {
            const int tap = k0 / d.Cin;
            const int ci0 = k0 - tap * d.Cin;
            const int ky = tap / 3, kx = tap - ky * 3;
#pragma unroll
            for (int j = 0; j < AV; j++) {
                const int iy = apy[j] + ky - 1, ix = apx[j] + kx - 1;
                const bool ok = (unsigned)iy < (unsigned)d.H && (unsigned)ix < (unsigned)d.W;
                pa[j] = ok ? *reinterpret_cast<const f32x4v*>(arow_ptr[j] + ((int64_t)iy * d.W + ix) * d.Cin + ci0 + akq * 4)
                           : f32x4v{0.f, 0.f, 0.f, 0.f};
            }
// ... 15 lines not shown
                if (n0 + nn + 2 < d.N) v.z = src[2];
                if (n0 + nn + 3 < d.N) v.w = src[3];
            }
            pb[j] = v;
        }
    };
    auto commit_from = [&](int buf, const f32x4v (&src)[AV]) {
        float* a = As + buf * TG_BK * TG_LDA;
#pragma unroll
        for (int j = 0; j < AV; j++) {
            const int r = ar + AROWS * j;
            a[(akq * 4 + 0) * TG_LDA + r] = src[j].x;
            a[(akq * 4 + 1) * TG_LDA + r] = src[j].y;
            a[(akq * 4 + 2) * TG_LDA + r] = src[j].z;
            a[(akq * 4 + 3) * TG_LDA + r] = src[j].w;
        }
        float* b = Bs + buf * TG_BK * BN;
#pragma unroll
        for (int j = 0; j < BV; j++) {
            const int idx = tid + 256 * j;
            const int kk = idx / (BN / 4), nn = (idx % (BN / 4)) * 4;
            *reinterpret_cast<f32x4v*>(&b[kk * BN + nn]) = pb[j];
        }
    };
    auto commit = [&](int buf) { commit_from(buf, pa); };

    f32x16 acc[2][NTW];
#pragma unroll
    for (int t = 0; t < NTW; t++) {
        const int col = n0 + wn * (BN / 2) + t * 32 + l31;
        const float bv = (bias && col < d.N) ? bias[col] : 0.0f;
#pragma unroll
        for (int r = 0; r < 16; r++) { acc[0][t][r] = bv; acc[1][t][r] = bv; }
    }

    const int nchunks = d.K / TG_BK;
    auto compute = [&](int buf) {
        const float* a = As + buf * TG_BK * TG_LDA + wm * 64 + l31;
        const float* b = Bs + buf * TG_BK * BN + wn * (BN / 2) + l31;
#pragma unroll
        for (int kp = 0; kp < TG_BK / 2; kp++) {
            const int kr = 2 * kp + half;
            const float a0 = a[kr * TG_LDA], a1 = a[kr * TG_LDA + 32];
#pragma unroll
            for (int t = 0; t < NTW; t++) {
                const float bt = b[kr * BN + t * 32];
                acc[0][t] = __builtin_amdgcn_mfma_f32_32x32x2f32(a0, bt, acc[0][t], 0, 0, 0);
                acc[1][t] = __builtin_amdgcn_mfma_f32_32x32x2f32(a1, bt, acc[1][t], 0, 0, 0);
            }
        }
    };
    if (PAIR) {
        prefetch_a_pair(0);
        prefetch_b_fast(0);
        commit_from(0, pa);
        __syncthreads();
        for (int c = 0; c < nchunks; c += 2) {
            prefetch_b_fast((c + 1) * TG_BK);
            compute(0);
            commit_from(1, pa2);
            __syncthreads();
            const bool more = c + 2 < nchunks;
            if (more) {
                prefetch_a_pair((c + 2) * TG_BK);
                prefetch_b_fast((c + 2) * TG_BK);
            }
            compute(1);
            if (more) commit_from(0, pa);
            __syncthreads();
        }
    } else {
        prefetch(0);
        commit(0);
        __syncthreads();
        for (int c = 0; c < nchunks; c++) {
            const int buf = c & 1;
            if (c + 1 < nchunks) prefetch((c + 1) * TG_BK);
            compute(buf);
            if (c + 1 < nchunks) commit(buf ^ 1);
            __syncthreads();
        }
    }

    if (n0 + BN <= d.N && (d.ldc & 3) == 0 && (((uintptr_t)C) & 15) == 0) {
        static_assert(4 * 32 * (BN / 2) <= 2 * TG_BK * TG_LDA + 2 * TG_BK * BN, "staging must fit the operand tiles");
        store_tile_rows<NTW>(acc, lds + wave * (32 * (BN / 2)), lane, d.relu != 0, C + n0 + wn * (BN / 2), m0 + wm * 64, d.M, d.ldc);
        return;
    }
#pragma unroll
    for (int i = 0; i < 2; i++)
#pragma unroll
        for (int t = 0; t < NTW; t++) {
            const int col = n0 + wn * (BN / 2) + t * 32 + l31;
            if (col >= d.N) continue;
#pragma unroll
            for (int r = 0; r < 16; r++) {
                const int64_t rr = m0 + wm * 64 + i * 32 + (r & 3) + 8 * (r >> 2) + 4 * half;
                if (rr >= d.M) continue;
                float v = acc[i][t][r];
                if (d.relu) v = v > 0.0f ? v : 0.0f;
                C[rr * d.ldc + col] = v;
            }
        }
}

template <int BN>
static void launch_gemm_tiled(const GemmDesc& d, hipStream_t s) {
    dim3 grid((unsigned)((d.M + TG_BM - 1) / TG_BM), (unsigned)((d.N + BN - 1) / BN), (unsigned)(d.batch > 0 ? d.batch : 1));
    size_t lds = (size_t)(2 * TG_BK * TG_LDA + 2 * TG_BK * BN) * sizeof(float);
    const bool pair = !d.im2col && (d.K % (2 * TG_BK)) == 0 && (d.ldb & 3) == 0 && (((uintptr_t)d.B) & 15) == 0 &&
                      (d.strideB & 3) == 0 && (d.N & 3) == 0 && d.N >= 4;
    if (d.im2col) hipLaunchKernelGGL((gemm_tiled_kernel<BN, true, false>), grid, dim3(256), lds, s, d);
    else if (pair && grid.y > 1) {
        GemmDesc e = d;
        e.nfast = 1; e.nx = (int)grid.x; e.ny = (int)grid.y;
        const dim3 g1((unsigned)((grid.x + 7) / 8 * 8 * grid.y), 1, grid.z);
        hipLaunchKernelGGL((gemm_tiled_kernel<BN, false, true>), g1, dim3(256), lds, s, e);
    } else if (pair) hipLaunchKernelGGL((gemm_tiled_kernel<BN, false, true>), grid, dim3(256), lds, s, d);
    else hipLaunchKernelGGL((gemm_tiled_kernel<BN, false, false>), grid, dim3(256), lds, s, d);
}

template <int NP>
__global__ void __launch_bounds__(256, NP == 3 ? 2 : 3) gemm_split_kernel(GemmDesc d) {
    extern __shared__ __attribute__((aligned(16))) float lds[];
    constexpr int PL = split::PLANE;
    float* As = lds;
    float* Bs = lds + 2 * NP * PL;
    const int tid = threadIdx.x, lane = tid & 63, wave = tid >> 6;
    const int half = lane >> 5, l31 = lane & 31;
    const int wm = wave >> 1, wn = wave & 1;
    const int z = blockIdx.z;
    const float* __restrict__ A = d.A + (int64_t)z * d.strideA;
    const float* __restrict__ bias = d.bias ? d.bias + (int64_t)z * d.strideBias : nullptr;
    float* __restrict__ C = d.C + (int64_t)z * d.strideC;
    const int xcd = blockIdx.x & 7, q = blockIdx.x >> 3;
    const int nblk = q % d.ny;
    const int mblk = (q / d.ny) * 8 + xcd;
    if (mblk >= d.nx) return;
    const int64_t m0 = (int64_t)mblk * split::BM;
    const int n0 = nblk * split::BN;
    const int nchunks = d.K / split::BK;
    const float* __restrict__ img = reinterpret_cast<const float*>(d.Bsplit + (int64_t)z * d.strideBsplit) +
                                    (int64_t)nblk * nchunks * split::image_floats;
    const int ar = tid >> 2, akq = tid & 3;
    const float* arow[2];
#pragma unroll
    for (int j = 0; j < 2; j++) {
        int64_t row = m0 + ar + 64 * j;
        if (row >= d.M) row = d.M - 1;
        arow[j] = A + row * d.lda + akq * 4;
    }
    split::f32x16s acc[2][2];
#pragma unroll
    for (int t = 0; t < 2; t++) {
        const int col = n0 + wn * 64 + t * 32 + l31;
        const float bv = bias ? bias[col] : 0.0f;
#pragma unroll
        for (int r = 0; r < 16; r++) { acc[0][t][r] = bv; acc[1][t][r] = bv; }
    }
    split::pipeline<NP>(nchunks,
        [&](int k0, split::f32x4s (&d0)[2], split::f32x4s (&d1)[2]) {
#pragma unroll
            for (int j = 0; j < 2; j++) {
                d0[j] = *reinterpret_cast<const split::f32x4s*>(arow[j] + k0);
                d1[j] = *reinterpret_cast<const split::f32x4s*>(arow[j] + k0 + split::BK);
            }
        },
        [&](int k0, int ring) { split::load_weights<NP>(img + (int64_t)(k0 / split::BK) * split::image_floats, Bs + ring * NP * PL, wave, lane); },
        [&](int abuf, const split::f32x4s (&v)[2]) {
            char* base = reinterpret_cast<char*>(As + abuf * NP * PL);
#pragma unroll
            for (int j = 0; j < 2; j++) split::commit4<NP>(base, ar + 64 * j, akq, v[j][0], v[j][1], v[j][2], v[j][3]);
        },
        [&](int abuf, int ring) {
            split::mma_chunk<NP>(reinterpret_cast<const char*>(As + abuf * NP * PL), reinterpret_cast<const char*>(Bs + ring * NP * PL),
                                 wm, wn, l31, half, acc);
        });
    if ((d.ldc & 3) == 0 && (((uintptr_t)C) & 15) == 0) {
        store_tile_rows<2>(acc, lds + wave * (32 * 64), lane, d.relu != 0, C + n0 + wn * 64, m0 + wm * 64, d.M, d.ldc);
        return;
    }
#pragma unroll
    for (int i = 0; i < 2; i++)
#pragma unroll
        for (int t = 0; t < 2; t++) {
            const int col = n0 + wn * 64 + t * 32 + l31;
#pragma unroll
            for (int r = 0; r < 16; r++) {
                const int64_t rr = m0 + wm * 64 + i * 32 + (r & 3) + 8 * (r >> 2) + 4 * half;
                if (rr >= d.M) continue;
                float v = acc[i][t][r];
                if (d.relu) v = v > 0.0f ? v : 0.0f;
                C[rr * d.ldc + col] = v;
            }
        }
}

static bool launch_gemm_split(const GemmDesc& d, int numerics, hipStream_t s) {
    if (!d.Bsplit || d.im2col || d.convt || (d.K % 64) != 0 || (d.N % 128) != 0 || (d.lda & 3) != 0 || (((uintptr_t)d.A) & 15) != 0 ||
        (d.strideA & 3) != 0 || d.M < 1) return false;
    GemmDesc e = d;
    e.nx = (int)((d.M + split::BM - 1) / split::BM);
// ... 462 lines not shown
    hipLaunchKernelGGL(sigmoid_kernel, dim3(grid), dim3(256), 0, s, x, y, count);
}

__global__ void __launch_bounds__(256)
conv1x1_cout1_kernel(const float* __restrict__ x, int64_t pixels, int cin, const float* __restrict__ wt,
                     const float* __restrict__ bias, int relu, int do_sigmoid, float* __restrict__ y) {
    for (int64_t p = (int64_t)blockIdx.x * blockDim.x + threadIdx.x; p < pixels; p += (int64_t)gridDim.x * blockDim.x) {
        float acc = bias[0];
        const float* xp = x + p * cin;
        if ((cin & 3) == 0) {
            for (int c = 0; c < cin; c += 4) {
                float4 v = *reinterpret_cast<const float4*>(xp + c);
                acc = fmaf(v.x, wt[c], acc);
                acc = fmaf(v.y, wt[c + 1], acc);
                acc = fmaf(v.z, wt[c + 2], acc);
                acc = fmaf(v.w, wt[c + 3], acc);
            }
        } else {
            for (int c = 0; c < cin; c++) acc = fmaf(xp[c], wt[c], acc);
        }
        if (relu) acc = acc > 0.0f ? acc : 0.0f;
        y[p] = do_sigmoid ? spec_sigmoidf(acc) : acc;
    }
}

void conv1x1_cout1(const float* x, int64_t pixels, int cin, const float* wt, const float* bias, int relu, int do_sigmoid,
                   float* y, hipStream_t s) {
    int grid = (int)((pixels + 255) / 256 < 16384 ? (pixels + 255) / 256 : 16384);
    if (grid < 1) grid = 1;
    hipLaunchKernelGGL(conv1x1_cout1_kernel, dim3(grid), dim3(256), 0, s, x, pixels, cin, wt, bias, relu, do_sigmoid, y);
}

__global__ void __launch_bounds__(256) to_seq_kernel(const float* __restrict__ x, int n, int w, int c, float* __restrict__ y) {
    const int64_t total = (int64_t)n * w * c;
    for (int64_t i = (int64_t)blockIdx.x * blockDim.x + threadIdx.x; i < total; i += (int64_t)gridDim.x * blockDim.x) {
        const int ch = (int)(i % c);
        const int64_t r = i / c;
        const int b = (int)(r % n);
        const int t = (int)(r / n);
        y[i] = x[((int64_t)b * w + t) * c + ch];
    }
}

void to_seq(const float* x, int n, int w, int c, float* y, hipStream_t s) {
    int64_t total = (int64_t)n * w * c;
    int grid = (int)((total + 255) / 256 < 16384 ? (total + 255) / 256 : 16384);
    if (grid < 1) grid = 1;
    hipLaunchKernelGGL(to_seq_kernel, dim3(grid), dim3(256), 0, s, x, n, w, c, y);
}

__global__ void __launch_bounds__(256)
gru_gates_kernel(const float* __restrict__ gx, const float* __restrict__ gh, float* __restrict__ h,
                 float* __restrict__ y, int T, int N, int H, int step) {
    const int dir = blockIdx.y;
    const int t = dir ? T - 1 - step : step;
    const int64_t total = (int64_t)N * H;
    const float* gxp = gx + (int64_t)dir * T * N * 3 * H + (int64_t)t * N * 3 * H;
    const float* ghp = gh + (int64_t)dir * N * 3 * H;
    float* hp = h + (int64_t)dir * N * H;
    for (int64_t i = (int64_t)blockIdx.x * blockDim.x + threadIdx.x; i < total; i += (int64_t)gridDim.x * blockDim.x) {
        const int j = (int)(i % H);
        const int64_t b = i / H;
        const float* gxr = gxp + b * 3 * H;
        const float* ghr = ghp + b * 3 * H;
        float r = spec_sigmoidf(gxr[j] + ghr[j]);
        float z = spec_sigmoidf(gxr[H + j] + ghr[H + j]);
        float nn = spec_tanhf(fmaf(r, ghr[2 * H + j], gxr[2 * H + j]));
        float hprev = hp[i];
        float hn = fmaf(z, hprev - nn, nn);
        hp[i] = hn;
        y[((int64_t)t * N + b) * 2 * H + (int64_t)dir * H + j] = hn;
    }
}

void gru_gates(const float* gx, const float* gh, float* h, float* y, int T, int N, int H, int step, hipStream_t s) {
    int64_t total = (int64_t)N * H;
    int grid = (int)((total + 255) / 256 < 4096 ? (total + 255) / 256 : 4096);
    if (grid < 1) grid = 1;
    hipLaunchKernelGGL(gru_gates_kernel, dim3(grid, 2), dim3(256), 0, s, gx, gh, h, y, T, N, H, step);
}

constexpr int LSM_ROWS = 64;

__device__ __forceinline__ void log_softmax_argmax_body(const float* __restrict__ logits, int64_t rows, int c,
                                                        const uint8_t* __restrict__ excl, float* __restrict__ logp,
                                                        int32_t* __restrict__ labels, float* __restrict__ maxlp) {
    extern __shared__ float tile[];
    const int cp = (c & 1) ? c : c + 1;
    const int64_t r0 = (int64_t)blockIdx.x * LSM_ROWS;
    const int nrows = (int)min((int64_t)LSM_ROWS, rows - r0);
    for (int i = threadIdx.x; i < nrows * c; i += LSM_ROWS) {
        int rr = i / c, cc = i - rr * c;
        tile[rr * cp + cc] = logits[r0 * c + i];
    }
    __syncthreads();
    if ((int)threadIdx.x < nrows) {
        float* row = tile + threadIdx.x * cp;
        float m = row[0];
        for (int j = 1; j < c; j++) m = row[j] > m ? row[j] : m;
        float ssum = 0.0f;
        for (int j = 0; j < c; j++) ssum = ssum + spec_expf(row[j] - m);
        const float lse = m + spec_logf(ssum);
        const float ninf = -__builtin_huge_valf();
        int best = 0;
        float bv = row[0] - lse;
        row[0] = bv;
        if (excl && excl[0]) bv = ninf;
        for (int j = 1; j < c; j++) {
            float v = row[j] - lse;
            row[j] = v;
            if (excl && excl[j]) v = ninf;
            if (v > bv) { bv = v; best = j; }
        }
        if (labels) labels[r0 + threadIdx.x] = best;
        if (maxlp) maxlp[r0 + threadIdx.x] = bv;
    }
    __syncthreads();
    if (logp)
        for (int i = threadIdx.x; i < nrows * c; i += LSM_ROWS) {
            int rr = i / c, cc = i - rr * c;
            logp[r0 * c + i] = tile[rr * cp + cc];
        }
}

__global__ void __launch_bounds__(LSM_ROWS)
log_softmax_argmax_kernel(const float* __restrict__ logits, int64_t rows, int c, const uint8_t* __restrict__ excl,
                          float* __restrict__ logp, int32_t* __restrict__ labels) {
    log_softmax_argmax_body(logits, rows, c, excl, logp, labels, nullptr);
}

__global__ void __launch_bounds__(LSM_ROWS)
log_softmax_argmax_max_kernel(const float* __restrict__ logits, int64_t rows, int c, const uint8_t* __restrict__ excl,
                              float* __restrict__ logp, int32_t* __restrict__ labels, float* __restrict__ maxlp) {
    log_softmax_argmax_body(logits, rows, c, excl, logp, labels, maxlp);
}

bool log_softmax_argmax(const float* logits, int64_t rows, int c, const uint8_t* d_excluded, float* logp,
                        int32_t* labels, hipStream_t s, float* maxlp) {
    if (rows <= 0) return true;
    int cp = (c & 1) ? c : c + 1;
    size_t lds = (size_t)LSM_ROWS * cp * sizeof(float);
    if (lds > 160 * 1024) return false;
    if (lds > 64 * 1024) {
        static std::atomic<uint64_t> lds_ok{0}, lds_ok_max{0};
        if (maxlp) allow_dynamic_lds(reinterpret_cast<const void*>(&log_softmax_argmax_max_kernel), lds_ok_max);
        else allow_dynamic_lds(reinterpret_cast<const void*>(&log_softmax_argmax_kernel), lds_ok);
    }
    int grid = (int)((rows + LSM_ROWS - 1) / LSM_ROWS);
    if (maxlp)
        hipLaunchKernelGGL(log_softmax_argmax_max_kernel, dim3(grid), dim3(LSM_ROWS), lds, s, logits, rows, c, d_excluded,
                           logp, labels, maxlp);
    else
        hipLaunchKernelGGL(log_softmax_argmax_kernel, dim3(grid), dim3(LSM_ROWS), lds, s, logits, rows, c, d_excluded, logp,
                           labels);
    return true;
}

__global__ void __launch_bounds__(256)
to_seq_packed_kernel(const float* __restrict__ x, int n, int T, int c, const int32_t* __restrict__ pos,
                     const int32_t* __restrict__ off, float* __restrict__ y) {
    const int64_t total = (int64_t)n * T * c;
    for (int64_t i = (int64_t)blockIdx.x * blockDim.x + threadIdx.x; i < total; i += (int64_t)gridDim.x * blockDim.x) {
        const int ch = (int)(i % c);
        const int64_t r = i / c;
        const int t = (int)(r % T);
        const int line = (int)(r / T);
        y[((int64_t)off[t] + pos[line]) * c + ch] = x[i];
    }
}

void to_seq_packed(const float* x, int n, int T, int c, const int32_t* d_pos, const int32_t* d_off, float* y,
                   hipStream_t s) {
    int64_t total = (int64_t)n * T * c;
    if (total <= 0) return;
    int grid = (int)((total + 255) / 256 < 16384 ? (total + 255) / 256 : 16384);
    hipLaunchKernelGGL(to_seq_packed_kernel, dim3(grid), dim3(256), 0, s, x, n, T, c, d_pos, d_off, y);
}

__global__ void __launch_bounds__(256)
gru_gates_packed_kernel(const float* __restrict__ gx, const float* __restrict__ gh, float* __restrict__ h,
                        float* __restrict__ y, const int32_t* __restrict__ Tm, const int32_t* __restrict__ off,
                        int64_t R, int Mcap, int active, int H, int step) {
    const int dir = blockIdx.y;
    const int64_t total = (int64_t)active * H;
    const float* gxd = gx + (int64_t)dir * R * 3 * H;
    const float* ghd = gh + (int64_t)dir * Mcap * 3 * H;
    float* hd = h + (int64_t)dir * Mcap * H;
    for (int64_t i = (int64_t)blockIdx.x * blockDim.x + threadIdx.x; i < total; i += (int64_t)gridDim.x * blockDim.x) {
        const int j = (int)(i % H);
        const int m = (int)(i / H);
        const int t = dir ? Tm[m] - 1 - step : step;
        const int64_t row = (int64_t)off[t] + m;
        const float* gxr = gxd + row * 3 * H;
        const float* ghr = ghd + (int64_t)m * 3 * H;
        float r = spec_sigmoidf(gxr[j] + ghr[j]);
        float z = spec_sigmoidf(gxr[H + j] + ghr[H + j]);
// ... 71 lines not shown
        const float br = bhd[j0 + i16], bz = bhd[H + j0 + i16], bn = bhd[2 * H + j0 + i16];
        for (int r = 0; r < 4; r++) { acc_r[r] = br; acc_z[r] = bz; acc_n[r] = bn; }
    }
    const float* bp = &lds_w[kq * 48 + i16];
#pragma unroll
    for (int s4 = 0; s4 < H / 4; s4++) {
        const float a = areg[s4];
        const float* b = bp + s4 * 4 * 48;
        acc_r = __builtin_amdgcn_mfma_f32_16x16x4f32(a, b[0], acc_r, 0, 0, 0);
        acc_z = __builtin_amdgcn_mfma_f32_16x16x4f32(a, b[16], acc_z, 0, 0, 0);
        acc_n = __builtin_amdgcn_mfma_f32_16x16x4f32(a, b[32], acc_n, 0, 0, 0);
    }
    float hnew[4];
#pragma unroll
    for (int r = 0; r < 4; r++) {
        float hn = 0.0f;
        if (rok[r]) {
            const float rg = spec_sigmoidf(gxr_[r] + acc_r[r]);
            const float zg = spec_sigmoidf(gxz_[r] + acc_z[r]);
            const float ng = spec_tanhf(fmaf(rg, acc_n[r], gxn_[r]));
            hn = fmaf(zg, hprev_[r] - ng, ng);
            y[yrow[r] * 2 * H + (int64_t)dir * H + j] = hn;
        }
        hnew[r] = hn;
    }
    float* hp = hout + (int64_t)j * Mcap + mbase;
    if (mbase + 3 < Mcap) {
        *reinterpret_cast<float4*>(hp) = make_float4(hnew[0], hnew[1], hnew[2], hnew[3]);
    } else {
        for (int r = 0; r < 4 && mbase + r < Mcap; r++) hp[r] = hnew[r];
    }
}

bool gru_step_fused(const float* gx, const float* wh, const float* bh, const float* hT_in, float* hT_out, float* y,
                    const int32_t* d_Tm, const int32_t* d_off, int64_t R, int Mcap, int active, int H, int step,
                    hipStream_t s) {
    if (active <= 0) return true;
    dim3 grid((active + 63) / 64, H / 16, 2);
    size_t lds = (size_t)H * 48 * sizeof(float);
    if (H == 256)
        hipLaunchKernelGGL((gru_step_fused_kernel<256>), grid, dim3(256), lds, s, gx, wh, bh, hT_in, hT_out, y, d_Tm, d_off,
                           R, Mcap, active, step);
    else if (H == 128)
        hipLaunchKernelGGL((gru_step_fused_kernel<128>), grid, dim3(256), lds, s, gx, wh, bh, hT_in, hT_out, y, d_Tm, d_off,
                           R, Mcap, active, step);
    else if (H == 64)
        hipLaunchKernelGGL((gru_step_fused_kernel<64>), grid, dim3(256), lds, s, gx, wh, bh, hT_in, hT_out, y, d_Tm, d_off, R,
                           Mcap, active, step);
    else
        return false;
    return true;
}

void gru_gates_packed(const float* gx, const float* gh, float* h, float* y, const int32_t* d_Tm, const int32_t* d_off,
                      int64_t R, int Mcap, int active, int H, int step, hipStream_t s) {
    int64_t total = (int64_t)active * H;
    if (total <= 0) return;
    int grid = (int)((total + 255) / 256 < 4096 ? (total + 255) / 256 : 4096);
    hipLaunchKernelGGL(gru_gates_packed_kernel, dim3(grid, 2), dim3(256), 0, s, gx, gh, h, y, d_Tm, d_off, R, Mcap, active,
                       H, step);
}

__global__ void __launch_bounds__(64)
ctc_collapse_packed_kernel(const int32_t* __restrict__ labels, const int32_t* __restrict__ Tm,
                           const int32_t* __restrict__ off, int M, int Tmax, uint32_t* __restrict__ out_labels,
                           uint32_t* __restrict__ out_pos, int32_t* __restrict__ out_count) {
    const int m = blockIdx.x * blockDim.x + threadIdx.x;
    if (m >= M) return;
    const int T = Tm[m];
    int last = 0, cnt = 0;
    for (int t = 0; t < T; t++) {
        int l = labels[(int64_t)off[t] + m];
        if (l == last) continue;
        last = l;
        if (l > 0) {
            out_labels[(int64_t)m * Tmax + cnt] = (uint32_t)l;
            out_pos[(int64_t)m * Tmax + cnt] = (uint32_t)t;
            cnt++;
        }
    }
    out_count[m] = cnt;
}

void ctc_collapse_packed(const int32_t* labels, const int32_t* d_Tm, const int32_t* d_off, int M, int Tmax,
                         uint32_t* out_labels, uint32_t* out_pos, int32_t* out_count, hipStream_t s) {
    if (M <= 0) return;
    hipLaunchKernelGGL(ctc_collapse_packed_kernel, dim3((M + 63) / 64), dim3(64), 0, s, labels, d_Tm, d_off, M, Tmax,
                       out_labels, out_pos, out_count);
}

constexpr int CTC_U = 16;

__global__ void __launch_bounds__(64)
ctc_collapse_scored_packed_kernel(const int32_t* __restrict__ labels, const float* __restrict__ maxlp,
                                  const int32_t* __restrict__ Tm, const int32_t* __restrict__ off, int M, int Tmax,
                                  uint32_t* __restrict__ out_labels, uint32_t* __restrict__ out_pos,
                                  float* __restrict__ out_logp, int32_t* __restrict__ out_count,
                                  double* __restrict__ out_score) {
    const int m = blockIdx.x * blockDim.x + threadIdx.x;
    const int T = m < M ? Tm[m] : 0;
    int Tw = T;
#pragma unroll
    for (int d = 32; d >= 1; d >>= 1) Tw = max(Tw, __shfl_xor(Tw, d));
    int last = 0, cnt = 0;
    double s = 0.0;
    const int64_t base = (int64_t)m * Tmax;
    for (int t0 = 0; t0 < Tw; t0 += CTC_U) {
        int l[CTC_U];
        float v[CTC_U];
#pragma unroll
        for (int u = 0; u < CTC_U; u++) {
            const int t = t0 + u;
            l[u] = 0;
            v[u] = 0.0f;
            if (t < T) {
                const int64_t r = (int64_t)off[t] + m;
                l[u] = labels[r];
                v[u] = maxlp[r];
            }
        }
#pragma unroll
        for (int u = 0; u < CTC_U; u++) {
            const int t = t0 + u;
            if (t >= T) break;
            s += (double)v[u];
            if (l[u] == last) continue;
            last = l[u];
            if (l[u] > 0) {
                out_labels[base + cnt] = (uint32_t)l[u];
                out_pos[base + cnt] = (uint32_t)t;
                out_logp[base + cnt] = v[u];
                cnt++;
            }
        }
    }
    if (m < M) {
        out_count[m] = cnt;
        out_score[m] = s;
    }
}

void ctc_collapse_scored_packed(const int32_t* labels, const float* maxlp, const int32_t* d_Tm, const int32_t* d_off, int M,
                                int Tmax, uint32_t* out_labels, uint32_t* out_pos, float* out_logp, int32_t* out_count,
                                double* out_score, hipStream_t s) {
    if (M <= 0) return;
    hipLaunchKernelGGL(ctc_collapse_scored_packed_kernel, dim3((M + 63) / 64), dim3(64), 0, s, labels, maxlp, d_Tm, d_off, M,
                       Tmax, out_labels, out_pos, out_logp, out_count, out_score);
}

__global__ void __launch_bounds__(256)
argmax_rows_kernel(const float* __restrict__ x, int64_t rows, int c, const uint8_t* __restrict__ excl,
                   int32_t* __restrict__ labels) {
    for (int64_t r = (int64_t)blockIdx.x * blockDim.x + threadIdx.x; r < rows; r += (int64_t)gridDim.x * blockDim.x) {
        const float* row = x + r * c;
        const float ninf = -__builtin_huge_valf();
        int best = 0;
        float bv = (excl && excl[0]) ? ninf : row[0];
        for (int j = 1; j < c; j++) {
            float v = (excl && excl[j]) ? ninf : row[j];
            if (v > bv) { bv = v; best = j; }
        }
        labels[r] = best;
    }
}

void argmax_rows(const float* x, int64_t rows, int c, const uint8_t* d_excluded, int32_t* labels, hipStream_t s) {
    if (rows <= 0) return;
    int grid = (int)((rows + 255) / 256 < 4096 ? (rows + 255) / 256 : 4096);
    hipLaunchKernelGGL(argmax_rows_kernel, dim3(grid), dim3(256), 0, s, x, rows, c, d_excluded, labels);
// ... 31 lines not shown
```

### ocrs_amd/csrc/model.hpp

```cpp
#pragma once
#include <functional>
#include <memory>
#include <string>
#include <vector>

#include "common.hpp"

namespace ocrs {

enum OpType : uint32_t {
    OP_CONV = 0, OP_DWCONV3, OP_MAXPOOL, OP_AVGPOOL, OP_CONVT2, OP_PADCAT, OP_SIGMOID, OP_TOSEQ, OP_GRU, OP_LINEAR,
    OP_LOGSOFTMAX, OP_COUNT
};

struct GraphOp {
    uint32_t type;
    int32_t in0, in1, out;
    int32_t relu, kh, kw, cin, cout, hidden;
    const float* w[8] = {nullptr};
    size_t wcount[8] = {0};
    const float* aux0 = nullptr;
    const float* aux1 = nullptr;
    const float* aux2 = nullptr;
    const float* aux3 = nullptr;
// ... 5 lines not shown
    bool cat_into_next = false;
    bool reads_cat = false;
    int dc_block = -1;
};

struct DcBlock {
    int first = -1, last = -1;
    int convt = -1, cat = -1, dw1 = -1, pw1 = -1, dw2 = -1, pw2 = -1, pool = -1, fin = -1, sig = -1;
    int cs = 0, cx = 0, cmid = 0, cout = 0;
    const float* tape = nullptr;
    int tape_len = 0;
    const float* rtape = nullptr;
    int rtape_len = 0;
};

struct TensorShape {
    int n = 0, h = 0, w = 0, c = 0;
    bool seq = false;
    int64_t count() const { return (int64_t)n * h * w * c; }
};

struct ModelBase {
    virtual ~ModelBase() = default;
    int device = -1;
    int64_t input_shape[4] = {-1, -1, -1, -1};
    virtual bool is_callback() const = 0;
};

struct CallbackModel : ModelBase {
    ocrs_model_run_fn fn = nullptr;
    void* user = nullptr;
    bool is_callback() const override { return true; }
    void run(const float* input, const int64_t in_shape[4], std::vector<float>& out, int64_t out_shape[4],
             int* out_ndim) const;
};

struct HipModel : ModelBase {
    uint32_t kind = 0;
    std::vector<GraphOp> ops;
    std::vector<DcBlock> dc_blocks;
    uint32_t n_slots = 0, out_slot = 0;
    DevBuf weights;
    std::vector<DevBuf> tapes;
    bool is_callback() const override { return false; }

    static std::unique_ptr<HipModel> load(const void* data, size_t len, int device = -1);

    TensorShape infer(int n, int h, int w, std::vector<TensorShape>* slots = nullptr) const;
    double flops(int n, int h, int w) const;

    float* run_device(Workspace& ws, const float* d_in, int n, int h, int w, TensorShape* out_shape,
                      StageTimers* timers, const uint8_t* d_excluded = nullptr, int32_t* d_labels = nullptr,
                      bool want_logp = true, bool print_timing = false, int stop_before = -1,
                      hipStream_t exec = nullptr ) const;

    int packed_split() const;
    struct PackedGroup {
        const float* d_batch;
        int n, w;
        const int32_t* d_pos;
    };
    struct PackedPlan {
        int M = 0, Tmax = 0;
        int64_t R = 0;
        const int32_t* d_Tm = nullptr;
        const int32_t* d_off = nullptr;
        std::vector<int> active;
        std::vector<int32_t> h_Tm;
        std::vector<int32_t> h_off;
        uint32_t* h_status = nullptr;
    };
    struct OpRange {
        int first = 0, last = 0;
        bool gx_only = false;
        const float* seq_in = nullptr;
        int in_c = 0;
        const float* out = nullptr;
        int out_c = 0;
    };
    static const int32_t* make_packed_plan(Workspace& ws, const std::vector<int32_t>& T, PackedPlan* plan, std::vector<size_t>* order);
    int run_recognition_packed(Workspace& ws, const std::vector<PackedGroup>& groups, const PackedPlan& plan, int h,
                               StageTimers* timers, const uint8_t* d_excluded, int32_t* d_labels,
                               float** d_logp = nullptr, float* d_maxlp = nullptr, OpRange* range = nullptr) const;
    float* run_prefix_ragged(Workspace& ws, hipStream_t exec, const std::vector<PackedGroup>& groups,
                             const PackedPlan& plan, int h, int ts, StageTimers* timers, int* feat_c,
                             const std::function<void()>& before_launch = nullptr, const OpRange* range = nullptr,
                             hipEvent_t* stack_done = nullptr) const;
};

}

struct ocrs_model {
    std::unique_ptr<ocrs::ModelBase> impl;
};
```

### ocrs_amd/csrc/model_packed.cpp

```cpp
#include <functional>
#include <mutex>

#include "model_exec.hpp"
#include "ragged_plan.hpp"

namespace ocrs {

namespace {
bool ragged_stack_supported(const std::vector<GraphOp>& ops, int ts, int h) {
    for (int i = 0; i < ts; i++) {
        const GraphOp& op = ops[i];
        if (op.in0 != (i == 0 ? 0 : ops[i - 1].out)) return false;
        if (op.type == OP_CONV) {
            if (op.kh != 3 || op.kw != 3 || !op.relu) return false;
            if (op.cin == 1) {
                if (i + 1 >= ts || ops[i + 1].type != OP_MAXPOOL || ops[i + 1].kh != 2 || ops[i + 1].kw != 2) return false;
                if (op.cout > 64 || op.cout < 4 || (op.cout & (op.cout - 1)) != 0) return false;
            } else if ((op.cin % 32) != 0 || op.cout < 64 || (op.cout % 4) != 0) {
                return false;
            }
        } else if (op.type != OP_MAXPOOL && op.type != OP_AVGPOOL) {
            return false;
        }
    }
// ... 319 lines not shown
                ran = np ? k::gru_persistent_split(gx, op.aux2, op.aux3, y, static_cast<uint16_t*>(hx), plan.d_Tm, plan.d_off, plan.h_Tm.data(), R, M, plan.Tmax, H, np, d_sync, rs)
                         : k::gru_persistent(gx, op.aux2, op.aux3, y, static_cast<float*>(hx), plan.d_Tm, plan.d_off, plan.h_Tm.data(), R, M, plan.Tmax, H, d_sync, rs);
            });
            if (ran && plan.h_status && gru_layer < 8)
                ws.download(plan.h_status + gru_layer, d_sync + k::gru_persistent_sync_words(M) - 1, sizeof(uint32_t), rs);
            OCRS_HIP(hipEventRecord(done, rs));
            if (rs == st || ws.stream.may_park_waits()) OCRS_HIP(hipStreamWaitEvent(st, done, 0));
            else rec_done = done;
        }
        if (rec_done) ws.host_wait(rec_done);
        return ran;
    }

    void gru_steps_fused(const GraphOp& op, const float* gx, float* y) {
        const int H = op.hidden, Mcap = (plan.M + 3) & ~3;
        float* hT0 = ws.alloc_n<float>((size_t)2 * H * Mcap);
        float* hT1 = ws.alloc_n<float>((size_t)2 * H * Mcap);
        OCRS_HIP(hipMemsetAsync(hT0, 0, (size_t)2 * H * Mcap * sizeof(float), st));
        for (int step = 0; step < plan.Tmax; step++) {
            const int act = plan.active[step];
            if (act <= 0) break;
            const float* hin = (step & 1) ? hT1 : hT0;
            float* hout = (step & 1) ? hT0 : hT1;
            timed(KC_GEMM_GRU_HIDDEN, 2.0 * 2 * act * 3.0 * H * H,
                  4.0 * 2 * ((double)act * H * 2 + (double)act * 3 * H + 3.0 * H * H + (double)act * H), [&] {
                      if (!k::gru_step_fused(gx, op.aux2, op.aux3, hin, hout, y, plan.d_Tm, plan.d_off, plan.R, Mcap, act, H, step, st))
                          fail(OCRS_ERR_RUN_FAILED, "model run failed: no fused GRU step kernel for hidden size %d", H);
                  });
        }
    }

    void gru_steps_unfused(const GraphOp& op, const float* gx, float* y) {
        const int H = op.hidden, M = plan.M;
        float* gh = ws.alloc_n<float>((size_t)2 * M * 3 * H);
        float* hs = ws.alloc_n<float>((size_t)2 * M * H);
        OCRS_HIP(hipMemsetAsync(hs, 0, (size_t)2 * M * H * sizeof(float), st));
        k::GemmDesc r = desc::gru_hidden(op, hs, gh, M);
        for (int step = 0; step < plan.Tmax; step++) {
            const int act = plan.active[step];
            if (act <= 0) break;
            r.M = act;
            timed(KC_GEMM_GRU_HIDDEN, 2.0 * 2 * act * (double)r.N * r.K,
                  4.0 * 2 * ((double)act * r.K + (double)act * r.N + (double)r.K * r.N), [&] { k::gemm(r, st); });
            timed(KC_GRU_GATES, 0, 4.0 * 2 * act * (double)H * 9,
                  [&] { k::gru_gates_packed(gx, gh, hs, y, plan.d_Tm, plan.d_off, plan.R, M, act, H, step, st); });
        }
    }

    bool run_gru_layer(const GraphOp& op, bool is_last) {
        const int H = op.hidden, I = op.cin, M = plan.M;
        const int64_t R = plan.R;
        if (I != curC) fail(OCRS_ERR_RUN_FAILED, "model run failed: GRU input size %d != %d", I, curC);
        int tok = begin(ST_REC_GRU);
        const size_t gx_floats = (size_t)2 * R * 3 * H;
        if (gx_floats > gx_cap) { gx_buf = ws.alloc_n<float>(gx_floats); gx_cap = gx_floats; }
        float* gx = gx_buf;
        float* y = ws.alloc_n<float>((size_t)R * 2 * H);
        const bool fused = (H == 256 || H == 128 || H == 64);
        const bool persistent = fused && gru_mode() == GRU_PERSISTENT && k::gru_persistent_supported(plan.h_Tm.data(), M, plan.Tmax, R, H);
        int np = option(OPT_NUMERICS) == 1 ? 3 : option(OPT_NUMERICS) == 2 ? 2 : 0;
        if (!(persistent && np != 0 && k::gru_split_supported(plan.h_Tm.data(), M, plan.Tmax, R, H, np))) np = 0;
        const size_t hx_bytes = np ? k::gru_split_exchange_bytes(plan.h_Tm.data(), M, H, np) : persistent ? k::gru_persistent_exchange_bytes(plan.h_Tm.data(), M, H) : 0;
        if (hx_bytes > hx_cap) { hx_buf = ws.alloc(hx_bytes); hx_cap = hx_bytes; }
        if (np) OCRS_HIP(k::gru_split_prepare(static_cast<uint16_t*>(hx_buf), plan.h_Tm.data(), M, H, np, st));
        else if (persistent) OCRS_HIP(k::gru_persistent_prepare(static_cast<float*>(hx_buf), plan.h_Tm.data(), M, H, st));
        const k::GemmDesc d = desc::gru_input(op, cur, gx, R, true);
        timed(KC_GEMM_GRU_INPUT, 2.0 * 2 * R * (double)d.N * d.K, 4.0 * ((double)R * I + 2.0 * R * d.N + 2.0 * d.K * d.N),
              [&] { k::gemm(d, st); });
        if (range && range->gx_only && is_last) {
            range->out = gx; range->out_c = 3 * H;
            return false;
        }
        if (!(persistent && gru_persistent_launch(op, gx, y, hx_buf, np))) {
            if (fused) gru_steps_fused(op, gx, y);
            else gru_steps_unfused(op, gx, y);
        }
        end(tok);
        gru_layer++;
        cur = y;
        curC = 2 * H;
        return true;
    }

    void run_linear(const GraphOp& op) {
        const int64_t R = plan.R;
        if (op.cin != curC) fail(OCRS_ERR_RUN_FAILED, "model run failed: Linear input size %d != %d", op.cin, curC);
        int tok = begin(ST_REC_HEAD);
        float* y = ws.alloc_n<float>((size_t)R * op.cout);
        const k::GemmDesc d = desc::dense(op, cur, y, R);
        timed(KC_GEMM_LINEAR, 2.0 * R * (double)d.N * d.K, 4.0 * ((double)R * (op.cin + op.cout)) + 4.0 * op.wcount[0],
              [&] { k::gemm(d, st); });
        end(tok);
        cur = y;
        curC = op.cout;
    }

    int run_log_softmax(const uint8_t* d_excluded, int32_t* d_labels, float** d_logp, float* d_maxlp) {
        const int64_t R = plan.R;
        int tok = begin(ST_REC_HEAD);
        float* lp = nullptr;
        if (d_logp || range) {
            lp = ws.alloc_n<float>((size_t)R * curC);
            if (d_logp) *d_logp = lp;
        }
        timed(KC_LOGSOFTMAX_ARGMAX, 0, 4.0 * R * curC * (lp ? 2.0 : 1.0), [&] {
            if (!k::log_softmax_argmax(cur, R, curC, d_excluded, lp, d_labels, st, d_maxlp))
                fail(OCRS_ERR_CAPACITY, "LogSoftmax over %d classes exceeds the kernel's LDS staging (max ~630)", curC);
        });
        end(tok);
        if (range) cur = lp;
        return curC;
    }
};
}

int HipModel::run_recognition_packed(Workspace& ws, const std::vector<PackedGroup>& groups, const PackedPlan& plan, int h,
                                     StageTimers* timers, const uint8_t* d_excluded, int32_t* d_labels,
                                     float** d_logp, float* d_maxlp, OpRange* range) const {
    const int ts = packed_split();
    if (ts < 0) fail(OCRS_ERR_RUN_FAILED, "model run failed: graph is not <conv stack> TOSEQ GRU* LINEAR LOGSOFTMAX");
    const int first = range ? range->first : 0, last = range ? range->last : (int)ops.size() - 1;
    PackedRun run{*this, ws, plan, timers, range, ws.s()};
    if (first <= ts) {
        int C0 = 0;
        float* X = run.run_conv_stack(groups, h, ts, &C0);
        if (range) {
            if (!X) fail(OCRS_ERR_INVALID_ARGUMENT, "op range: this model's conv stack has no ragged form");
            if (last < ts) {
                range->out = X; range->out_c = C0;
                return 0;
            }
        }
        if (!X) X = run.run_groups_unpacked(groups, h, ts, &C0);
        if (!X) return 0;
        run.cur = X; run.curC = C0;
    } else {
        run.cur = range->seq_in; run.curC = range->in_c;
    }
    int classes = 0;
    for (int i = std::max(ts + 1, first); i <= last; i++) {
        const GraphOp& op = ops[i];
        if (op.type == OP_LINEAR) run.run_linear(op);
        else if (op.type == OP_LOGSOFTMAX) classes = run.run_log_softmax(d_excluded, d_labels, d_logp, d_maxlp);
        else if (!run.run_gru_layer(op, i == last)) return 0;
    }
    if (range) { range->out = run.cur; range->out_c = run.curC; }
    OCRS_HIP(hipGetLastError());
    return classes;
}

}
```

Measured before the change: 285.5.

## Fuse recognition head linear GEMM with log-softmax argmax and wave-level CTC collapse

When only labels (and optionally max log-prob) are needed, the final Linear GEMM now runs a HEAD variant that writes the output tile to LDS and computes the log-softmax and argmax in the epilogue. This removes the separate logits buffer and the log-softmax kernel launch. CTC collapse also gets a wave-per-line kernel that uses ballot and popcount instead of one thread per line. The fused epilogue adds LDS staging and syncs to the GEMM and runs the per-row reduction serially on one wave, which may slow the GEMM tail.

```diff
diff --git a/include/ocrs_amd.h b/include/ocrs_amd.h
--- a/include/ocrs_amd.h
+++ b/include/ocrs_amd.h
@@ -364,6 +364,12 @@
                                                      int last_op, int gx_only, const float* input, size_t input_len, float** out,
                                                      size_t** out_offsets, int32_t** out_shapes);
 
+OCRS_API ocrs_status ocrs_engine_run_recognition_head(const ocrs_engine* e, const float* x, size_t rows, size_t in_features,
+                                                      size_t classes, const uint8_t* excluded, int32_t* labels, float* maxlp, float* logp,
+                                                      int* fused);
+OCRS_API ocrs_status ocrs_engine_ctc_collapse(const ocrs_engine* e, const int32_t* lengths, size_t n_lines, const int32_t* labels,
+                                              uint32_t** out_labels, uint32_t** out_pos, size_t** out_offsets);
+
 OCRS_API ocrs_status ocrs_text_item_rotated_rect(const int32_t* rects_tlbr, size_t n_chars, float out6[6]);
 OCRS_API ocrs_status ocrs_rotated_rect_corners(const float rect6[6], float out8[8]);
 
diff --git a/ocrs_amd/__init__.py b/ocrs_amd/__init__.py
--- a/ocrs_amd/__init__.py
+++ b/ocrs_amd/__init__.py
@@ -1216,6 +1216,35 @@
         lib().ocrs_buffer_free(shp)
         return res
 
+    def run_recognition_head(self, x, classes, excluded=None, maxlp=False, logp=False):
+        a = np.ascontiguousarray(x, np.float32)
+        rows, k = a.shape
+        classes = int(classes)
+        ex = None if excluded is None else np.ascontiguousarray(excluded, np.uint8)
+        if ex is not None and ex.shape != (classes,):
+            raise ValueError("excluded: expected %d flags" % classes)
+        labels = np.zeros(rows, np.int32)
+        mx = np.zeros(rows, np.float32) if maxlp else None
+        lp = np.zeros((rows, classes), np.float32) if logp else None
+        fused = C.c_int(0)
+        check(lib().ocrs_engine_run_recognition_head(
+            self._h, a.ctypes.data_as(C.POINTER(C.c_float)), C.c_size_t(rows), C.c_size_t(k), C.c_size_t(classes),
+            ex.ctypes.data_as(C.POINTER(C.c_uint8)) if ex is not None else None, labels.ctypes.data_as(C.POINTER(C.c_int32)),
+            mx.ctypes.data_as(C.POINTER(C.c_float)) if maxlp else None, lp.ctypes.data_as(C.POINTER(C.c_float)) if logp else None,
+            C.byref(fused)))
+        return {"labels": labels, "maxlp": mx, "logp": lp, "fused": bool(fused.value)}
+
+    def ctc_collapse(self, lines):
+        lens = np.ascontiguousarray([len(l) for l in lines], np.int32)
+        flat = np.ascontiguousarray(np.concatenate([np.asarray(l, np.int32).ravel() for l in lines] + [np.zeros(0, np.int32)]), np.int32)
+        lab, pos, offs = C.POINTER(C.c_uint32)(), C.POINTER(C.c_uint32)(), C.POINTER(C.c_size_t)()
+        check(lib().ocrs_engine_ctc_collapse(self._h, lens.ctypes.data_as(C.POINTER(C.c_int32)), C.c_size_t(len(lens)),
+                                             flat.ctypes.data_as(C.POINTER(C.c_int32)), C.byref(lab), C.byref(pos), C.byref(offs)))
+        out = [[(int(lab[k]), int(pos[k])) for k in range(offs[i], offs[i + 1])] for i in range(len(lens))]
+        for p in (lab, pos, offs):
+            lib().ocrs_buffer_free(p)
+        return out
+
     def prepare_recognition_input(self, inp, line, rectify=False):
         a = _rects_to_array(line)
         out = C.POINTER(C.c_float)()
diff --git a/ocrs_amd/_lib.py b/ocrs_amd/_lib.py
--- a/ocrs_amd/_lib.py
+++ b/ocrs_amd/_lib.py
@@ -66,7 +66,7 @@
     "ocrs_group_member_stats", "ocrs_numa_parse_cpulist", "ocrs_numa_bind_selftest", "ocrs_engine_recognize_logits", "ocrs_engine_set_option", "ocrs_engine_get_option", "ocrs_option_name", "ocrs_device_pool_stats", "ocrs_device_pool_configure", "ocrs_device_pool_trim",
     "ocrs_device_set_isolation", "ocrs_device_isolation", "ocrs_group_set_replay", "ocrs_abi_version",
     "ocrs_engine_recognize_text_scored", "ocrs_engine_recognize_text_batch_scored", "ocrs_ctc_beam_search_scored",
-    "ocrs_engine_run_recognition_ops",
+    "ocrs_engine_run_recognition_ops", "ocrs_engine_run_recognition_head", "ocrs_engine_ctc_collapse",
     "ocrs_engine_detect_words_scored", "ocrs_engine_detect_words_batch_scored", "ocrs_group_detect_words_batch_scored",
     "ocrs_engine_find_text_lines_indexed", "ocrs_engine_find_text_lines_batch_indexed",
     "ocrs_detection_tile_plan", "ocrs_engine_detect_words_tiled", "ocrs_engine_detect_words_batch_tiled",
diff --git a/ocrs_amd/csrc/abi.cpp b/ocrs_amd/csrc/abi.cpp
--- a/ocrs_amd/csrc/abi.cpp
+++ b/ocrs_amd/csrc/abi.cpp
@@ -955,6 +955,27 @@
     });
 }
 
+ocrs_status ocrs_engine_run_recognition_head(const ocrs_engine* e, const float* x, size_t rows, size_t in_features,
+                                             size_t classes, const uint8_t* excluded, int32_t* labels, float* maxlp, float* logp, int* fused) {
+    return guarded_engine(e, [&] {
+        if (!e || !x || !labels || !fused) fail(OCRS_ERR_INVALID_ARGUMENT, "null argument");
+        *fused = e->run_recognition_head(x, rows, in_features, classes, excluded, labels, maxlp, logp) ? 1 : 0;
+    });
+}
+
+ocrs_status ocrs_engine_ctc_collapse(const ocrs_engine* e, const int32_t* lengths, size_t n_lines, const int32_t* labels,
+                                     uint32_t** out_labels, uint32_t** out_pos, size_t** out_offsets) {
+    return guarded_engine(e, [&] {
+        if (!e || (n_lines && !lengths) || !out_labels || !out_pos || !out_offsets) fail(OCRS_ERR_INVALID_ARGUMENT, "null argument");
+        std::vector<uint32_t> lab, pos;
+        std::vector<size_t> offs;
+        e->ctc_collapse(lengths, n_lines, labels, &lab, &pos, &offs);
+        *out_labels = dup_buffer(lab);
+        *out_pos = dup_buffer(pos);
+        *out_offsets = dup_buffer(offs);
+    });
+}
+
 ocrs_status ocrs_text_item_rotated_rect(const int32_t* rects_tlbr, size_t n_chars, float out6[6]) {
     return guarded([&] {
         if (!rects_tlbr || !out6 || n_chars == 0) fail(OCRS_ERR_INVALID_ARGUMENT, "expected valid rect");
diff --git a/ocrs_amd/csrc/common.cpp b/ocrs_amd/csrc/common.cpp
--- a/ocrs_amd/csrc/common.cpp
+++ b/ocrs_amd/csrc/common.cpp
@@ -500,12 +500,23 @@
 }
 int option(Option o) { return (int)option_long(o); }
 int conv_rows_setting() { return t_tuning ? (int)__atomic_load_n(&t_tuning->conv_rows, __ATOMIC_RELAXED) : (int)kConvRowsDefault; }
+int head_fuse_setting() { return t_tuning ? (int)__atomic_load_n(&t_tuning->head_fuse, __ATOMIC_RELAXED) : 1; }
+int collapse_form_setting() { return t_tuning ? (int)__atomic_load_n(&t_tuning->collapse_form, __ATOMIC_RELAXED) : 1; }
+
+namespace {
+long* switch_setting(Tuning& t, const char* name) {
+    if (name && strcmp(name, "head_fuse") == 0) return &t.head_fuse;
+    if (name && strcmp(name, "collapse_form") == 0) return &t.collapse_form;
+    return nullptr;
+}
+}
 
 Tuning default_tuning() {
     std::call_once(g_opts_once, init_options);
     Tuning t;
     for (int i = 0; i < OPT_COUNT; i++) t.v[i] = g_opts[i].load(std::memory_order_relaxed);
     t.conv_rows = kConvRowsDefault;
+    t.head_fuse = t.collapse_form = 1;
     return t;
 }
 
@@ -530,6 +541,11 @@
         __atomic_store_n(&t.conv_rows, value, __ATOMIC_RELAXED);
         return 0;
     }
+    if (long* sw = switch_setting(t, name)) {
+        if (value < 0 || value > 1) return 2;
+        __atomic_store_n(sw, value, __ATOMIC_RELAXED);
+        return 0;
+    }
     const int i = find_option(name, OPT_COUNT);
     if (i < 0) return 1;
     if (i == OPT_STREAM_BUDGET) return 4;
@@ -541,6 +557,10 @@
 bool get_option(const Tuning& t, const char* name, long* value) {
     if (name && strcmp(name, "conv_rows") == 0) {
         *value = __atomic_load_n(&t.conv_rows, __ATOMIC_RELAXED);
+        return true;
+    }
+    if (const long* sw = switch_setting(const_cast<Tuning&>(t), name)) {
+        *value = __atomic_load_n(sw, __ATOMIC_RELAXED);
         return true;
     }
     const int i = name && strcmp(name, "numerics") == 0 ? (int)OPT_NUMERICS : find_option(name, OPT_COUNT);
diff --git a/ocrs_amd/csrc/common.hpp b/ocrs_amd/csrc/common.hpp
--- a/ocrs_amd/csrc/common.hpp
+++ b/ocrs_amd/csrc/common.hpp
@@ -154,8 +154,10 @@
               OPT_LAYOUT_THREADS, OPT_REC_MAX_PIXELS,
               OPT_COUNT };
 constexpr long kConvRowsDefault = 2;
-struct Tuning { long v[OPT_COUNT]; long conv_rows; };
+struct Tuning { long v[OPT_COUNT]; long conv_rows; long head_fuse; long collapse_form; };
 int conv_rows_setting();
+int head_fuse_setting();
+int collapse_form_setting();
 Tuning default_tuning();
 int set_option(const char* name, long value);
 int set_option(Tuning& t, const char* name, long value);
diff --git a/ocrs_amd/csrc/engine.cpp b/ocrs_amd/csrc/engine.cpp
--- a/ocrs_amd/csrc/engine.cpp
+++ b/ocrs_amd/csrc/engine.cpp
@@ -933,6 +933,83 @@
     }
 }
 
+bool ocrs_engine::run_recognition_head(const float* x, size_t rows, size_t in_features, size_t classes, const uint8_t* excl, int32_t* labels,
+                                       float* maxlp, float* logp) const {
+    if (!recognition) fail(OCRS_ERR_MODEL_NOT_LOADED, "Recognition model not loaded");
+    if (recognition->is_callback()) fail(OCRS_ERR_INVALID_ARGUMENT, "run_recognition_head needs a model of the fixed-graph executor");
+    const auto* hm = static_cast<const HipModel*>(recognition);
+    if (hm->packed_split() < 0) fail(OCRS_ERR_INVALID_ARGUMENT, "recognition graph is not <conv stack> TOSEQ GRU* LINEAR LOGSOFTMAX");
+    const GraphOp& lin = hm->ops[hm->ops.size() - 2];
+    if (rows == 0 || rows > (size_t)INT32_MAX) fail(OCRS_ERR_INVALID_ARGUMENT, "%zu rows", rows);
+    if (in_features != (size_t)lin.cin) fail(OCRS_ERR_INVALID_ARGUMENT, "the Linear reads %d features, not %zu", lin.cin, in_features);
+    const size_t C = (size_t)lin.cout;
+    if (classes != C) fail(OCRS_ERR_INVALID_ARGUMENT, "the model has %zu classes, not %zu", C, classes);
+    Workspace ws;
+    float* d_x = ws.alloc_n<float>(rows * in_features);
+    ws.upload(d_x, x, rows * in_features * sizeof(float));
+    uint8_t* d_excl = nullptr;
+    if (excl) {
+        d_excl = ws.alloc_n<uint8_t>(C);
+        ws.upload(d_excl, excl, C);
+    }
+    int32_t* d_labels = ws.alloc_n<int32_t>(rows);
+    float* d_maxlp = maxlp ? ws.alloc_n<float>(rows) : nullptr;
+    float* d_logp = nullptr;
+    const bool fused = hm->run_recognition_head(ws, d_x, (int64_t)rows, (int)in_features, d_excl, d_labels, logp ? &d_logp : nullptr, d_maxlp);
+    ws.download(labels, d_labels, rows * sizeof(int32_t));
+    if (maxlp) ws.download(maxlp, d_maxlp, rows * sizeof(float));
+    if (logp) ws.download(logp, d_logp, rows * C * sizeof(float));
+    ws.sync();
+    return fused;
+}
+
+void ocrs_engine::ctc_collapse(const int32_t* lengths, size_t n, const int32_t* labels, std::vector<uint32_t>* out_labels,
+                               std::vector<uint32_t>* out_pos, std::vector<size_t>* offsets) const {
+    out_labels->clear();
+    out_pos->clear();
+    offsets->assign(n + 1, 0);
+    std::vector<int32_t> T(lengths, lengths + n);
+    std::vector<size_t> line_at(n);
+    size_t total = 0;
+    for (size_t i = 0; i < n; i++) {
+        if (T[i] < 0) fail(OCRS_ERR_INVALID_ARGUMENT, "line %zu: length %d", i, T[i]);
+        line_at[i] = total;
+        total += (size_t)T[i];
+    }
+    Workspace ws;
+    HipModel::PackedPlan plan;
+    std::vector<size_t> order;
+    if (!HipModel::make_packed_plan(ws, T, &plan, &order)) return;
+    const int M = plan.M, Tmax = plan.Tmax;
+    std::vector<int32_t> packed((size_t)plan.R);
+    for (int m = 0; m < M; m++)
+        for (int t = 0; t < T[order[m]]; t++) packed[(size_t)plan.h_off[t] + m] = labels[line_at[order[m]] + t];
+    int32_t* d_labels = ws.alloc_n<int32_t>(packed.size());
+    ws.upload(d_labels, packed.data(), packed.size() * sizeof(int32_t));
+    uint32_t* d_ol = ws.alloc_n<uint32_t>((size_t)M * Tmax);
+    uint32_t* d_op = ws.alloc_n<uint32_t>((size_t)M * Tmax);
+    int32_t* d_cnt = ws.alloc_n<int32_t>(M);
+    k::ctc_collapse_packed(d_labels, plan.d_Tm, plan.d_off, M, Tmax, d_ol, d_op, d_cnt, ws.s());
+    OCRS_HIP(hipGetLastError());
+    std::vector<uint32_t> hl((size_t)M * Tmax), hp((size_t)M * Tmax);
+    std::vector<int32_t> hc(M);
+    ws.download(hl.data(), d_ol, hl.size() * sizeof(uint32_t));
+    ws.download(hp.data(), d_op, hp.size() * sizeof(uint32_t));
+    ws.download(hc.data(), d_cnt, hc.size() * sizeof(int32_t));
+    ws.sync();
+    std::vector<int> slot_of(n, -1);
+    for (int m = 0; m < M; m++) slot_of[order[m]] = m;
+    for (size_t i = 0; i < n; i++) {
+        const int m = slot_of[i];
+        if (m >= 0) {
+            if (hc[m] < 0 || hc[m] > T[i]) fail(OCRS_ERR_RUN_FAILED, "line %zu: %d kept steps of %d", i, hc[m], T[i]);
+            out_labels->insert(out_labels->end(), hl.begin() + (size_t)m * Tmax, hl.begin() + (size_t)m * Tmax + hc[m]);
+            out_pos->insert(out_pos->end(), hp.begin() + (size_t)m * Tmax, hp.begin() + (size_t)m * Tmax + hc[m]);
+        }
+        (*offsets)[i + 1] = out_labels->size();
+    }
+}
+
 namespace {
 
 struct Chunk { uint32_t gw; std::vector<size_t> members; int64_t off; float* ptr = nullptr; };
diff --git a/ocrs_amd/csrc/engine.hpp b/ocrs_amd/csrc/engine.hpp
--- a/ocrs_amd/csrc/engine.hpp
+++ b/ocrs_amd/csrc/engine.hpp
@@ -147,6 +147,10 @@
                           std::vector<std::vector<float>>* logp, int* classes) const;
     void run_recognition_ops(const int32_t* widths, size_t n, int first_op, int last_op, bool gx_only, const float* in,
                              size_t in_len, std::vector<float>* out, std::vector<int32_t>* shapes) const;
+    bool run_recognition_head(const float* x, size_t rows, size_t in_features, size_t classes, const uint8_t* excl, int32_t* labels, float* maxlp,
+                              float* logp) const;
+    void ctc_collapse(const int32_t* lengths, size_t n, const int32_t* labels, std::vector<uint32_t>* out_labels,
+                      std::vector<uint32_t>* out_pos, std::vector<size_t>* offsets) const;
 
     std::vector<ocrs::TextChar> text_line_from_result(const ocrs::RecResult& res, std::vector<float>* char_logp = nullptr) const;
 
diff --git a/ocrs_amd/csrc/kernels.hpp b/ocrs_amd/csrc/kernels.hpp
--- a/ocrs_amd/csrc/kernels.hpp
+++ b/ocrs_amd/csrc/kernels.hpp
@@ -71,8 +71,11 @@
     int batch; int64_t strideA, strideB, strideBias, strideC;
     int nfast = 0, nx = 0, ny = 0;
     const uint16_t* Bsplit = nullptr; int64_t strideBsplit = 0;
+    int32_t* head_labels = nullptr; float* head_maxlp = nullptr; const uint8_t* head_excl = nullptr;
 };
 void gemm(const GemmDesc& d, hipStream_t s);
+bool gemm_head_supported(const GemmDesc& d);
+bool gemm_head(const GemmDesc& d, hipStream_t s);
 void conv_direct(const float* x, int n, int h, int w, int cin, const float* wt, const float* bias, int kh, int kw,
                  int cout, int relu, float* y, hipStream_t s);
 void dwconv3x3(const float* x, int n, int h, int w, int c, const float* wt, const float* bias, int relu, float* y,
diff --git a/ocrs_amd/csrc/kernels_nn.hip b/ocrs_amd/csrc/kernels_nn.hip
--- a/ocrs_amd/csrc/kernels_nn.hip
+++ b/ocrs_amd/csrc/kernels_nn.hip
@@ -167,7 +167,9 @@
     }
 }
 
-template <int BN, bool IM2COL, bool PAIR>
+__device__ __forceinline__ void log_softmax_argmax_row(float* row, int c, const uint8_t* __restrict__ excl, int* best_out, float* bv_out);
+
+template <int BN, bool IM2COL, bool PAIR, bool HEAD = false>
 __global__ void __launch_bounds__(256, 4) gemm_tiled_kernel(GemmDesc d) {
     extern __shared__ __attribute__((aligned(16))) float lds[];
     constexpr int NTW = BN / 64;
@@ -349,6 +351,37 @@
         }
     }
 
+    if constexpr (HEAD) {
+        const int cp = (d.N & 1) ? d.N : d.N + 1;
+#pragma unroll
+        for (int i = 0; i < 2; i++) {
+#pragma unroll
+            for (int t = 0; t < NTW; t++) {
+                const int col = wn * (BN / 2) + t * 32 + l31;
+                if (col < d.N) {
+#pragma unroll
+                    for (int r = 0; r < 16; r++) {
+                        float v = acc[i][t][r];
+                        if (d.relu) v = v > 0.0f ? v : 0.0f;
+                        lds[(wm * 32 + (r & 3) + 8 * (r >> 2) + 4 * half) * cp + col] = v;
+                    }
+                }
+            }
+            __syncthreads();
+            if (wave == (int)((blockIdx.x + i) & 3)) {
+                const int64_t rr = m0 + (lane >> 5) * 64 + i * 32 + (lane & 31);
+                int best;
+                float bv;
+                log_softmax_argmax_row(lds + lane * cp, d.N, d.head_excl, &best, &bv);
+                if (rr < d.M) {
+                    d.head_labels[rr] = best;
+                    if (d.head_maxlp) d.head_maxlp[rr] = bv;
+                }
+            }
+            if (i == 0) __syncthreads();
+        }
+        return;
+    }
     if (n0 + BN <= d.N && (d.ldc & 3) == 0 && (((uintptr_t)C) & 15) == 0) {
         static_assert(4 * 32 * (BN / 2) <= 2 * TG_BK * TG_LDA + 2 * TG_BK * BN, "staging must fit the operand tiles");
         store_tile_rows<NTW>(acc, lds + wave * (32 * (BN / 2)), lane, d.relu != 0, C + n0 + wn * (BN / 2), m0 + wm * 64, d.M, d.ldc);
@@ -385,6 +418,22 @@
         hipLaunchKernelGGL((gemm_tiled_kernel<BN, false, true>), g1, dim3(256), lds, s, e);
     } else if (pair) hipLaunchKernelGGL((gemm_tiled_kernel<BN, false, true>), grid, dim3(256), lds, s, d);
     else hipLaunchKernelGGL((gemm_tiled_kernel<BN, false, false>), grid, dim3(256), lds, s, d);
+}
+
+bool gemm_head_supported(const GemmDesc& d) {
+    return !d.im2col && !d.convt && d.batch <= 1 && d.M > 0 && d.N >= 1 && d.N <= 128 && d.K >= TG_BK && (d.K % TG_BK) == 0 &&
+           (d.lda & 3) == 0 && (((uintptr_t)d.A) & 15) == 0 && !(d.Bsplit && option(OPT_NUMERICS) != 0);
+}
+
+bool gemm_head(const GemmDesc& d, hipStream_t s) {
+    if (!gemm_head_supported(d) || !d.head_labels) return false;
+    const dim3 grid((unsigned)((d.M + TG_BM - 1) / TG_BM), 1, 1);
+    const int cp = (d.N & 1) ? d.N : d.N + 1;
+    const size_t lds = std::max((size_t)(2 * TG_BK * TG_LDA + 2 * TG_BK * 128), (size_t)64 * cp) * sizeof(float);
+    const bool pair = (d.K % (2 * TG_BK)) == 0 && (d.ldb & 3) == 0 && (((uintptr_t)d.B) & 15) == 0 && (d.N & 3) == 0 && d.N >= 4;
+    if (pair) hipLaunchKernelGGL((gemm_tiled_kernel<128, false, true, true>), grid, dim3(256), lds, s, d);
+    else hipLaunchKernelGGL((gemm_tiled_kernel<128, false, false, true>), grid, dim3(256), lds, s, d);
+    return true;
 }
 
 template <int NP>
@@ -1013,6 +1062,28 @@
 
 constexpr int LSM_ROWS = 64;
 
+__device__ __forceinline__ void log_softmax_argmax_row(float* row, int c, const uint8_t* __restrict__ excl, int* best_out,
+                                                       float* bv_out) {
+    float m = row[0];
+    for (int j = 1; j < c; j++) m = row[j] > m ? row[j] : m;
+    float ssum = 0.0f;
+    for (int j = 0; j < c; j++) ssum = ssum + spec_expf(row[j] - m);
+    const float lse = m + spec_logf(ssum);
+    const float ninf = -__builtin_huge_valf();
+    int best = 0;
+    float bv = row[0] - lse;
+    row[0] = bv;
+    if (excl && excl[0]) bv = ninf;
+    for (int j = 1; j < c; j++) {
+        float v = row[j] - lse;
+        row[j] = v;
+        if (excl && excl[j]) v = ninf;
+        if (v > bv) { bv = v; best = j; }
+    }
+    *best_out = best;
+    *bv_out = bv;
+}
+
 __device__ __forceinline__ void log_softmax_argmax_body(const float* __restrict__ logits, int64_t rows, int c,
                                                         const uint8_t* __restrict__ excl, float* __restrict__ logp,
                                                         int32_t* __restrict__ labels, float* __restrict__ maxlp) {
@@ -1026,23 +1097,9 @@
     }
     __syncthreads();
     if ((int)threadIdx.x < nrows) {
-        float* row = tile + threadIdx.x * cp;
-        float m = row[0];
-        for (int j = 1; j < c; j++) m = row[j] > m ? row[j] : m;
-        float ssum = 0.0f;
-        for (int j = 0; j < c; j++) ssum = ssum + spec_expf(row[j] - m);
-        const float lse = m + spec_logf(ssum);
-        const float ninf = -__builtin_huge_valf();
-        int best = 0;
-        float bv = row[0] - lse;
-        row[0] = bv;
-        if (excl && excl[0]) bv = ninf;
-        for (int j = 1; j < c; j++) {
-            float v = row[j] - lse;
-            row[j] = v;
-            if (excl && excl[j]) v = ninf;
-            if (v > bv) { bv = v; best = j; }
-        }
+        int best;
+        float bv;
+        log_softmax_argmax_row(tile + threadIdx.x * cp, c, excl, &best, &bv);
         if (labels) labels[r0 + threadIdx.x] = best;
         if (maxlp) maxlp[r0 + threadIdx.x] = bv;
     }
@@ -1280,9 +1337,42 @@
     out_count[m] = cnt;
 }
 
+__global__ void __launch_bounds__(256)
+ctc_collapse_packed_wave_kernel(const int32_t* __restrict__ labels, const int32_t* __restrict__ Tm,
+                                const int32_t* __restrict__ off, int M, int Tmax, uint32_t* __restrict__ out_labels,
+                                uint32_t* __restrict__ out_pos, int32_t* __restrict__ out_count) {
+    const int lane = threadIdx.x & 63;
+    const int m = blockIdx.x * 4 + (threadIdx.x >> 6);
+    if (m >= M) return;
+    const int T = Tm[m];
+    const int64_t base = (int64_t)m * Tmax;
+    int carry = 0, cnt = 0;
+    for (int t0 = 0; t0 < T; t0 += 64) {
+        const int t = t0 + lane;
+        const int l = t < T ? labels[(int64_t)off[t] + m] : 0;
+        int prev = __shfl_up(l, 1);
+        if (lane == 0) prev = carry;
+        const bool keep = t < T && l != prev && l > 0;
+        const unsigned long long kept = __ballot(keep);
+        if (keep) {
+            const int at = cnt + __popcll(kept & ((1ull << lane) - 1ull));
+            out_labels[base + at] = (uint32_t)l;
+            out_pos[base + at] = (uint32_t)t;
+        }
+        cnt += __popcll(kept);
+        carry = __shfl(l, 63);
+    }
+    if (lane == 0) out_count[m] = cnt;
+}
+
 void ctc_collapse_packed(const int32_t* labels, const int32_t* d_Tm, const int32_t* d_off, int M, int Tmax,
                          uint32_t* out_labels, uint32_t* out_pos, int32_t* out_count, hipStream_t s) {
     if (M <= 0) return;
+    if (collapse_form_setting() != 0) {
+        hipLaunchKernelGGL(ctc_collapse_packed_wave_kernel, dim3((M + 3) / 4), dim3(256), 0, s, labels, d_Tm, d_off, M, Tmax,
+                           out_labels, out_pos, out_count);
+        return;
+    }
     hipLaunchKernelGGL(ctc_collapse_packed_kernel, dim3((M + 63) / 64), dim3(64), 0, s, labels, d_Tm, d_off, M, Tmax,
                        out_labels, out_pos, out_count);
 }
diff --git a/ocrs_amd/csrc/model.hpp b/ocrs_amd/csrc/model.hpp
--- a/ocrs_amd/csrc/model.hpp
+++ b/ocrs_amd/csrc/model.hpp
@@ -111,6 +111,8 @@
     int run_recognition_packed(Workspace& ws, const std::vector<PackedGroup>& groups, const PackedPlan& plan, int h,
                                StageTimers* timers, const uint8_t* d_excluded, int32_t* d_labels,
                                float** d_logp = nullptr, float* d_maxlp = nullptr, OpRange* range = nullptr) const;
+    bool run_recognition_head(Workspace& ws, const float* d_x, int64_t R, int in_c, const uint8_t* d_excluded, int32_t* d_labels,
+                              float** d_logp, float* d_maxlp) const;
     float* run_prefix_ragged(Workspace& ws, hipStream_t exec, const std::vector<PackedGroup>& groups,
                              const PackedPlan& plan, int h, int ts, StageTimers* timers, int* feat_c,
                              const std::function<void()>& before_launch = nullptr, const OpRange* range = nullptr,
diff --git a/ocrs_amd/csrc/model_packed.cpp b/ocrs_amd/csrc/model_packed.cpp
--- a/ocrs_amd/csrc/model_packed.cpp
+++ b/ocrs_amd/csrc/model_packed.cpp
@@ -425,10 +425,25 @@
         return true;
     }
 
-    void run_linear(const GraphOp& op) {
+    bool head_fused = false;
+
+    void run_linear(const GraphOp& op, int32_t* labels = nullptr, const uint8_t* d_excluded = nullptr, float* d_maxlp = nullptr) {
         const int64_t R = plan.R;
         if (op.cin != curC) fail(OCRS_ERR_RUN_FAILED, "model run failed: Linear input size %d != %d", op.cin, curC);
         int tok = begin(ST_REC_HEAD);
+        if (labels && head_fuse_setting() != 0) {
+            k::GemmDesc h = desc::dense(op, cur, nullptr, R);
+            h.head_labels = labels; h.head_maxlp = d_maxlp; h.head_excl = d_excluded;
+            if (k::gemm_head_supported(h)) {
+                timed(KC_GEMM_LINEAR, 2.0 * R * (double)h.N * h.K, 4.0 * ((double)R * (op.cin + 1)) + 4.0 * op.wcount[0],
+                      [&] { k::gemm_head(h, st); });
+                end(tok);
+                head_fused = true;
+                cur = nullptr;
+                curC = op.cout;
+                return;
+            }
+        }
         float* y = ws.alloc_n<float>((size_t)R * op.cout);
         const k::GemmDesc d = desc::dense(op, cur, y, R);
         timed(KC_GEMM_LINEAR, 2.0 * R * (double)d.N * d.K, 4.0 * ((double)R * (op.cin + op.cout)) + 4.0 * op.wcount[0],
@@ -440,6 +455,7 @@
 
     int run_log_softmax(const uint8_t* d_excluded, int32_t* d_labels, float** d_logp, float* d_maxlp) {
         const int64_t R = plan.R;
+        if (head_fused) return curC;
         int tok = begin(ST_REC_HEAD);
         float* lp = nullptr;
         if (d_logp || range) {
@@ -483,8 +499,11 @@
     int classes = 0;
     for (int i = std::max(ts + 1, first); i <= last; i++) {
         const GraphOp& op = ops[i];
-        if (op.type == OP_LINEAR) run.run_linear(op);
-        else if (op.type == OP_LOGSOFTMAX) classes = run.run_log_softmax(d_excluded, d_labels, d_logp, d_maxlp);
+        if (op.type == OP_LINEAR) {
+            const bool labels_only = !range && !d_logp && d_labels && i + 1 <= last && ops[i + 1].type == OP_LOGSOFTMAX;
+            if (labels_only) run.run_linear(op, d_labels, d_excluded, d_maxlp);
+            else run.run_linear(op);
+        } else if (op.type == OP_LOGSOFTMAX) classes = run.run_log_softmax(d_excluded, d_labels, d_logp, d_maxlp);
         else if (!run.run_gru_layer(op, i == last)) return 0;
     }
     if (range) { range->out = run.cur; range->out_c = run.curC; }
@@ -492,4 +511,19 @@
     return classes;
 }
 
-}
+bool HipModel::run_recognition_head(Workspace& ws, const float* d_x, int64_t R, int in_c, const uint8_t* d_excluded,
+                                    int32_t* d_labels, float** d_logp, float* d_maxlp) const {
+    if (packed_split() < 0) fail(OCRS_ERR_RUN_FAILED, "model run failed: graph is not <conv stack> TOSEQ GRU* LINEAR LOGSOFTMAX");
+    PackedPlan plan;
+    plan.R = R;
+    PackedRun run{*this, ws, plan, nullptr, nullptr, ws.s()};
+    run.cur = d_x; run.curC = in_c;
+    const GraphOp& lin = ops[ops.size() - 2];
+    if (d_logp) run.run_linear(lin);
+    else run.run_linear(lin, d_labels, d_excluded, d_maxlp);
+    run.run_log_softmax(d_excluded, d_labels, d_logp, d_maxlp);
+    OCRS_HIP(hipGetLastError());
+    return run.head_fused;
+}
+
+}
```

Result: no change. 284.7, median of 5 (-0.3%).
